# ultravideo/kvazzup

Measured on AMD Instinct MI355X. Metric: hevc_encode_decode_fps, higher is better.
Workload: dtype u8

## Files before the change

### kvazzup_amd/csrc/dec_parse.hip

```cpp
#include <chrono>
#include <cstdio>
#include <cstdlib>
#include <cstring>
#include "decoder.h"

namespace kvzx {

enum { PART_2Nx2N = 0, PART_2NxN, PART_Nx2N, PART_NxN, PART_2NxnU, PART_2NxnD, PART_nLx2N, PART_nRx2N };

namespace {

struct StateTabs { uint8_t next_mps[128], next_lps[128]; uint8_t next[128][2]; uint8_t lps[128][4]; uint32_t lpsn[128][4]; };
const StateTabs &state_tabs()
{
  static const StateTabs t = [] {
    StateTabs t;
    for (int s = 0; s < 128; s++) {
      int st = s >> 1, mps = s & 1;
      t.next_mps[s] = (uint8_t)(((st < 62 ? st + 1 : st) << 1) | mps);
      t.next_lps[s] = (uint8_t)((kNextLps[st] << 1) | (st == 0 ? mps ^ 1 : mps));
      t.next[s][0] = t.next_mps[s]; t.next[s][1] = t.next_lps[s];
      for (int q = 0; q < 4; q++) { t.lps[s][q] = kRangeLps[st][q]; const int n = __builtin_clz((uint32_t)kRangeLps[st][q]) - 23; t.lpsn[s][q] = ((uint32_t)kRangeLps[st][q] << n) | ((uint32_t)n << 16) | ((uint32_t)kRangeLps[st][q] << 24); }
    }
    return t;
  }();
  return t;
}
struct CabacRegs {
  const uint8_t *p = nullptr, *end = nullptr;
  uint64_t value = 0; int bits = 0;
  uint32_t range = 510; uint32_t past = 0;
  const StateTabs *st = nullptr;
  uint16_t *ctx = nullptr;
  static __attribute__((noinline)) uint32_t word_tail(const uint8_t *p, const uint8_t *end) { uint32_t w = 0; for (int i = 0; i < 4; i++) w = (w << 8) | (p + i < end ? p[i] : 0u); return w; }
  __attribute__((always_inline)) inline uint32_t word()
  {
    uint32_t w;
    if (__builtin_expect(p + 4 <= end, 1)) { memcpy(&w, p, 4); w = __builtin_bswap32(w); }
    else { w = word_tail(p, end); past++; }
    p += 4;
    return w;
  }
  __attribute__((always_inline)) inline void refill() { if (__builtin_expect(bits < 16, 0)) { value = (value << 32) | word(); bits += 32; } }
  bool overrun() const { return past > 3; }
  __attribute__((always_inline)) inline int bin(int ci)
  {
    const uint32_t s = ctx[ci];
    const uint32_t e = st->lpsn[s][(range >> 6) & 3];
    const uint32_t rmps = range - (e >> 24);
    const uint64_t scaled = (uint64_t)rmps << bits;
    const bool isl = value >= scaled;
    value -= isl ? scaled : 0;
    const uint32_t nm = (rmps >> 8) ^ 1u;
    range = isl ? (e & 0x1ffu) : (rmps << nm);
    bits -= (int)(isl ? ((e >> 16) & 15u) : nm);
    ctx[ci] = st->next[s][isl];
    refill();
    return (int)((s & 1u) ^ (uint32_t)isl);
  }
  __attribute__((always_inline)) inline int bypass()
  {
    bits--;
    const uint64_t scaled = (uint64_t)range << bits;
    int b = 0;
    if (value >= scaled) { value -= scaled; b = 1; }
    refill();
    return b;
  }
  __attribute__((always_inline)) inline uint32_t bypass_bits(int n)
  {
    uint32_t v = 0;
    while (n > 0) {
      const int m = n > 16 ? 16 : n;
      if (m <= 2) { for (int i = 0; i < m; i++) v = (v << 1) | (uint32_t)bypass(); }
      else {
        bits -= m;
        const uint64_t scaled = (uint64_t)range << bits;
        const uint64_t q = value / scaled;
        value -= q * scaled;
        v = (v << m) | (uint32_t)(q & 0xffffu);
        refill();
      }
      n -= m;
    }
    return v;
  }
  __attribute__((always_inline)) inline int terminate()
  {
    range -= 2;
    if (value >= ((uint64_t)range << bits)) return 1;
    if (range < 256) { range <<= 1; bits--; }
    refill();
    return 0;
  }
};
struct CabacDec : CabacRegs {
  const uint8_t *buf = nullptr;
  uint16_t ctx_store[CTX_COUNT];
  CabacDec() { ctx = ctx_store; }
  CabacDec(const CabacDec &) = delete;
  void load_ctx(const uint8_t *src) { for (int i = 0; i < CTX_COUNT; i++) ctx_store[i] = src[i]; }
  void save_ctx(uint8_t *dst) const { for (int i = 0; i < CTX_COUNT; i++) dst[i] = (uint8_t)ctx_store[i]; }
  void start(const uint8_t *b, size_t l)
  {
    buf = b; p = b; end = b + l; past = 0; st = &state_tabs(); range = 510; ctx = ctx_store;
    value = word(); bits = 32 - 9;
    refill();
  }
  size_t bytes_consumed() const { const size_t consumed_bits = (size_t)(p - buf) * 8 - (size_t)bits; return (consumed_bits + 7) >> 3; }
};

std::atomic<long> g_yields{0};

void parse_sao(CabacDec &c, SaoParams &p, const SaoParams *left, const SaoParams *up, bool luma, bool chroma)
{
  memset(&p, 0, sizeof(p));
  if (left && c.bin(CTX_SAO_MERGE)) { p = *left; return; }
  if (up && c.bin(CTX_SAO_MERGE)) { p = *up; return; }
  for (int ci = 0; ci < 3; ci++) {
    if (!(ci ? chroma : luma)) continue;
    if (ci < 2) p.type[ci] = (uint8_t)(c.bin(CTX_SAO_TYPE) ? (c.bypass() ? 2 : 1) : 0);
    else { p.type[2] = p.type[1]; p.eo_class[2] = p.eo_class[1]; }
    if (!p.type[ci]) continue;
    int a[4];
    for (int i = 0; i < 4; i++) { a[i] = 0; while (a[i] < 7 && c.bypass()) a[i]++; }
    if (p.type[ci] == 1) {
      for (int i = 0; i < 4; i++) if (a[i] && c.bypass()) a[i] = -a[i];
      p.band_pos[ci] = (uint8_t)c.bypass_bits(5);
    } else {
      if (ci < 2) p.eo_class[ci] = (uint8_t)c.bypass_bits(2);
      a[2] = -a[2]; a[3] = -a[3];
    }
    for (int i = 0; i < 4; i++) p.offset[ci][i] = (int8_t)a[i];
  }
}

__attribute__((noinline)) uint32_t sig_flag_run(CabacRegs &cr, const uint8_t *pk, int base, int k0)
{
  CabacRegs c = cr;
  uint32_t sig = 0;
  for (int k = k0; k >= 1; k--) sig |= (uint32_t)c.bin(base + pk[k]) << k;
  cr.p = c.p; cr.value = c.value; cr.bits = c.bits; cr.range = c.range; cr.past = c.past;
  return sig;
}
__attribute__((noinline)) uint32_t greater1_run(CabacRegs &cr, int ctx_base, int n, int *c1_io)
{
  CabacRegs c = cr;
  uint32_t g = 0; int c1 = *c1_io;
  for (int j = 0; j < n; j++) {
    const int g1 = c.bin(ctx_base + c1);
    g |= (uint32_t)g1 << j;
    if (g1) c1 = 0; else if (c1 > 0 && c1 < 3) c1++;
  }
  *c1_io = c1;
  cr.p = c.p; cr.value = c.value; cr.bits = c.bits; cr.range = c.range; cr.past = c.past;
  return g;
}

__attribute__((always_inline)) inline bool parse_residual_regs(CabacRegs &c, int log2, int cidx, int scan_idx, bool sign_hiding, bool ts_enabled, int *tskip, std::vector<uint32_t> &out)
{
  const ScanTabs &S = scan_tabs();
  const int n = 1 << log2, sbl = log2 - 2, nsb = 1 << sbl;
  const uint8_t *SX = S.x[scan_idx][sbl], *SY = S.y[scan_idx][sbl], *PX = S.x[scan_idx][2], *PY = S.y[scan_idx][2];
  uint8_t csbf[8][8]; memset(csbf, 0, sizeof(csbf));
  *tskip = (ts_enabled && log2 == 2) ? c.bin(CTX_TS_FLAG + (cidx ? 1 : 0)) : 0;
  int pre[2];
  for (int d = 0; d < 2; d++) {
    int off, sh, mx = (log2 << 1) - 1, v = 0;
    if (cidx == 0) { off = 3 * (log2 - 2) + ((log2 - 1) >> 2); sh = (log2 + 1) >> 2; } else { off = 15; sh = log2 - 2; }
    while (v < mx && c.bin((d ? CTX_LAST_Y : CTX_LAST_X) + off + (v >> sh))) v++;
    pre[d] = v;
  }
  int lx = pre[0], ly = pre[1];
  if (lx > 3) { int nb = (lx >> 1) - 1; lx = (1 << nb) * (2 + (lx & 1)) + (int)c.bypass_bits(nb); }
  if (ly > 3) { int nb = (ly >> 1) - 1; ly = (1 << nb) * (2 + (ly & 1)) + (int)c.bypass_bits(nb); }
  if (scan_idx == 2) { int tt = lx; lx = ly; ly = tt; }
  if (lx >= n || ly >= n) return false;
  const int last_sb = S.inv[scan_idx][sbl][((ly >> 2) << sbl) | (lx >> 2)], last_pos = S.inv[scan_idx][2][((ly & 3) << 2) | (lx & 3)];
  int c1 = 1;
  for (int i = last_sb; i >= 0; i--) {
    const int xs = SX[i], ys = SY[i];
    int right = (xs < nsb - 1) ? csbf[ys][xs + 1] : 0, below = (ys < nsb - 1) ? csbf[ys + 1][xs] : 0, infer_dc = 0;
    if (i < last_sb && i > 0) { csbf[ys][xs] = (uint8_t)c.bin(CTX_CSBF + ((right | below) ? 1 : 0) + (cidx ? 2 : 0)); infer_dc = 1; }
    else csbf[ys][xs] = 1;
    if (!csbf[ys][xs]) continue;
    uint32_t sig = 0;
    if (i == last_sb) sig |= 1u << last_pos;
    const int prev_csbf = right | (below << 1);
    const uint8_t *pk = S.sigk[scan_idx][log2 == 2 ? 4 : prev_csbf];
    const int sig_base = CTX_SIG + (cidx ? 27 : 0);
    const int sig_off = log2 == 2 ? 0 : (cidx == 0 ? ((i > 0 ? 3 : 0) + ((log2 == 3) ? ((scan_idx == 0) ? 9 : 15) : 21)) : ((log2 == 3) ? 9 : 12));
    {
      const int k0 = (i == last_sb) ? last_pos - 1 : 15;
      const int base = sig_base + sig_off;
      if (k0 >= 1) sig |= sig_flag_run(c, pk, base, k0);
      if (k0 >= 0) {
        if (infer_dc && !(sig >> 1)) sig |= 1u;
        else sig |= (uint32_t)c.bin((i == 0 && log2 != 2) ? sig_base : base + pk[0]);
      }
    }
    if (!sig) continue;
    int ctx_set = (i > 0 && cidx == 0) ? 2 : 0;
    if (c1 == 0) ctx_set++;
    c1 = 1;
    int pos[16], lev[16], nsig = 0, g1idx = -1;
    for (uint32_t m = sig; m;) { const int k = 31 - __builtin_clz(m); pos[nsig++] = k; m &= ~(1u << k); }
    for (int j = 0; j < nsig; j++) lev[j] = 1;
    {
      const uint32_t g = greater1_run(c, CTX_GT1 + (cidx ? 16 : 0) + ctx_set * 4, nsig < 8 ? nsig : 8, &c1);
      if (g) { g1idx = __builtin_ctz(g); for (uint32_t m = g; m; m &= m - 1) lev[__builtin_ctz(m)] = 2; }
    }
    if (g1idx >= 0 && c.bin(CTX_GT2 + (cidx ? 4 : 0) + ctx_set)) lev[g1idx] = 3;
    const bool hidden = sign_hiding && (pos[0] - pos[nsig - 1] > 3);
    const int nsigns = hidden ? nsig - 1 : nsig;
    uint32_t signs = c.bypass_bits(nsigns) << (nsig - nsigns);
    int rice = 0, sum = 0;
    for (int j = 0; j < nsig; j++) {
      int base = (j < 8) ? ((j == g1idx) ? 3 : 2) : 1;
      if (lev[j] == base) {
        int prefix = 0;
        while (prefix < 32 && c.bypass()) prefix++;
        if (prefix - 3 + rice > 16) return false;
        int rem = prefix <= 3 ? (prefix << rice) + (int)c.bypass_bits(rice)
                              : (((1 << (prefix - 3)) + 3 - 1) << rice) + (int)c.bypass_bits(prefix - 3 + rice);
        lev[j] = base + rem;
        if (lev[j] > 3 * (1 << rice)) rice = imin(rice + 1, 4);
      }
      sum += lev[j];
    }
    if (hidden && (sum & 1)) signs |= 1u;
    const size_t o0 = out.size();
    out.resize(o0 + (size_t)nsig);
    uint32_t *dst = out.data() + o0;
    for (int j = 0; j < nsig; j++) {
      const int v = ((signs >> (nsig - 1 - j)) & 1) ? -lev[j] : lev[j];
      const int xp = PX[pos[j]], yp = PY[pos[j]];
      dst[j] = (uint32_t)((((ys << 2) + yp) * n + (xs << 2) + xp) << 16) | ((uint32_t)clip3(-32768, 32767, v) & 0xffffu);
    }
    if (c.overrun()) return false;
  }
  return !c.overrun();
}

bool parse_residual(CabacDec &cd, int log2, int cidx, int scan_idx, bool sign_hiding, bool ts_enabled, int *tskip, std::vector<uint32_t> &out)
{
  CabacRegs c = cd;
  const bool ok = parse_residual_regs(c, log2, cidx, scan_idx, sign_hiding, ts_enabled, tskip, out);
  static_cast<CabacRegs &>(cd) = c;
  return ok;
}

struct MvCand { int mvx, mvy, ref_idx; };

struct SliceParser {
  Decoder::PicJob &job; Decoder::SubOut &out;
  const DecSps &sps; const DecPps &pps; const SliceHdr &sh;
  CabacDec c;
  const int w, h, b4w, b8w, ctbl, mincb, wc, hc;
  B4Rec *b4; uint8_t *pm, *ctd, *im;
  int ref_y0 = -(1 << 30), ref_y1 = 1 << 30;
  int tile_y0 = 0, tile_y1 = 1 << 30, tile_x0 = 0, tile_x1 = 1 << 30;
  const uint8_t *slice_of = nullptr; int cur_slice = 0;
  int slice_qp = 26;
  int err = 0;
  int qp_y = 0, qp_y_pred = 0, last_qp_y = 0, cu_qp_delta_val = 0, log2_qg = 6; bool qp_delta_coded = false;
  int cu_pred_mode = 0, part_mode = 0, max_trafo_depth = 0, intra_modes[4] = {0, 0, 0, 0}, chroma_mode = 0; bool intra_split = false;
  uint32_t ctu_intra_mask = 0;

  SliceParser(Decoder::PicJob &j, Decoder::SubOut &o, int pw)
      : job(j), out(o), sps(*j.sps), pps(j.pps), sh(j.sh), w(j.sps->width), h(j.sps->height), b4w(pw / 4), b8w(pw / 8), ctbl(j.sps->ctb_log2), mincb(j.sps->min_cb_log2), wc(j.sps->wc()),
        hc(j.sps->hc()), b4(j.b4), pm(j.pred_mode.data()), ctd(j.ct_depth.data()), im(j.intra_mode.data())
  { log2_qg = ctbl - pps.qp_delta_depth; }

  inline int bi(int x, int y) const { return (y >> 2) * b4w + (x >> 2); }
  inline int b8(int x, int y) const { return (y >> 3) * b8w + (x >> 3); }
  inline bool avail(int, int, int xn, int yn) const
  {
    return xn >= tile_x0 && yn >= tile_y0 && xn < w && yn < h && yn < tile_y1 && xn < tile_x1 && pm[b8(xn, yn)] != PM_NONE && (!slice_of || slice_of[(yn >> ctbl) * wc + (xn >> ctbl)] == cur_slice);
  }
  void fill_cu8(uint8_t *arr, int x0, int y0, int n, int v)
  {
    const int cols = imin(n, w - x0) >> 3;
    for (int y = y0; y < y0 + n && y < h; y += 8) memset(arr + b8(x0, y), v, (size_t)cols);
  }
  void fill_u8(uint8_t *arr, int x0, int y0, int bw, int bh, int v)
  {
    const int cols = imin(bw, w - x0) >> 2;
    for (int y = y0; y < y0 + bh && y < h; y += 4) memset(arr + bi(x0, y), v, (size_t)cols);
  }
  bool cu_edges_done = false;
  int cu_bypass = 0;
  void fill_recs(int x0, int y0, int bw, int bh, const B4Rec &r, bool cu_edges = false)
  {
    uint64_t v; memcpy(&v, &r, 8);
    const int cols = imin(bw, w - x0) >> 2;
    if (!cu_edges) { for (int y = y0; y < y0 + bh && y < h; y += 4) { uint64_t *p = (uint64_t *)&b4[bi(x0, y)]; for (int i = 0; i < cols; i++) p[i] = v; } return; }
    B4Rec e = r;
    e.flags |= B4_EDGE_V | B4_TU_V; uint64_t vl; memcpy(&vl, &e, 8);
    e.flags = r.flags | B4_EDGE_H | B4_TU_H; uint64_t vt; memcpy(&vt, &e, 8);
    e.flags |= B4_EDGE_V | B4_TU_V; uint64_t vc; memcpy(&vc, &e, 8);
    for (int y = y0; y < y0 + bh && y < h; y += 4) {
      uint64_t *p = (uint64_t *)&b4[bi(x0, y)];
      const bool top = y == y0;
      if (cols > 0) p[0] = top ? vc : vl;
      for (int i = 1; i < cols; i++) p[i] = top ? vt : v;
    }
    cu_edges_done = true;
  }
  void emit_tu(const DecTu &td)
  {
    const int X = td.plane ? td.x * 2 : td.x, Y = td.plane ? td.y * 2 : td.y;
    if (ctbl == 6) {
      TuRange &r = job.region[(Y >> 5) * (b4w >> 3) + (X >> 5)];
      if (!r.count) r.first = (uint32_t)out.tus.size();
      r.count++;
    }
    out.tus.push_back(td);
  }

  bool pb_avail(int xcb, int ycb, int ncbs, int xpb, int ypb, int npbw, int npbh, int part_idx, int xn, int yn) const
  {
    const bool same_cb = xcb <= xn && ycb <= yn && xcb + ncbs > xn && ycb + ncbs > yn;
    bool a;
    if (!same_cb) a = avail(xpb, ypb, xn, yn);
    else a = !((npbw << 1) == ncbs && (npbh << 1) == ncbs && part_idx == 1 && (ycb + npbh <= yn) && (xcb + npbw > xn));
    if (a && pm[b8(xn, yn)] == PM_INTRA) a = false;
    return a;
  }
  static bool same_motion(const B4Rec &a, const B4Rec &b) { return a.ref_idx == b.ref_idx && a.mvx == b.mvx && a.mvy == b.mvy; }

  inline int list_poc(int L, int idx) const { return L ? job.ref_poc1[idx & 15] : job.ref_poc[idx & 15]; }
  inline bool list_lt(int L, int idx) const { return (L ? job.ref_lt1[idx & 15] : job.ref_lt[idx & 15]) != 0; }
  static void scale_by(int &mvx, int &mvy, int td_, int tb_)
  {
    const int td = clip3(-128, 127, td_), tb = clip3(-128, 127, tb_);
    if (td == 0) return;
    const int tx = (16384 + (iabs(td) >> 1)) / td, dsf = clip3(-4096, 4095, (tb * tx + 32) >> 6);
    const int px = dsf * mvx, py = dsf * mvy;
    mvx = clip3(-32768, 32767, (px < 0 ? -1 : 1) * ((iabs(px) + 127) >> 8));
    mvy = clip3(-32768, 32767, (py < 0 ? -1 : 1) * ((iabs(py) + 127) >> 8));
  }
  bool temporal_mv(int xpb, int ypb, int npbw, int npbh, int X, int ref_idx, int &mvx, int &mvy)
  {
    ColMotion *col = job.col.get();
    if (!col) return false;
    const int cy = ypb >> ctbl;
    if (cy < col->hc) {
      std::atomic<uint8_t> &d = col->row_done[(size_t)cy];
      int spins = 0;
      while (!d.load(std::memory_order_acquire)) { if (++spins < 2000) __builtin_ia32_pause(); else std::this_thread::yield(); }
    }
    const int cand[2][2] = {{xpb + npbw, ypb + npbh}, {xpb + (npbw >> 1), ypb + (npbh >> 1)}};
    for (int k = 0; k < 2; k++) {
      int x = cand[k][0], y = cand[k][1];
      if (k == 0 && !((ypb >> ctbl) == (y >> ctbl) && y < h && x < w)) continue;
      x >>= 4; y >>= 4;
      if (x >= col->w16 || y >= col->h16) continue;
      const ColMotion::Mv &m = col->mv[(size_t)y * col->w16 + x];
      if (!m.used) continue;
      const int L = m.used == 2 ? 1 : (m.used == 1 ? 0 : (job.no_backward ? X : sh.collocated_from_l0));
      const bool cur_lt = list_lt(X, ref_idx);
      if ((((m.lt >> L) & 1) != 0) != cur_lt) continue;
      const int col_diff = col->poc - m.ref_poc[L], cur_diff = sh.poc - list_poc(X, ref_idx);
      mvx = m.mv[L][0]; mvy = m.mv[L][1];
      if (!cur_lt && col_diff != cur_diff && col_diff != 0) scale_by(mvx, mvy, col_diff, cur_diff);
      return true;
    }
    return false;
  }

  void merge_candidates(int xcb, int ycb, int ncbs, int xpb, int ypb, int npbw, int npbh, int part_idx, int pmode, MvCand *cand, int want)
  {
    const int lvl = pps.par_mrg_level;
    int n = 0;
    if (lvl > 2 && ncbs == 8) { xpb = xcb; ypb = ycb; npbw = npbh = ncbs; part_idx = 0; pmode = PART_2Nx2N; }
    auto par = [&](int xn, int yn) { return ((xpb >> lvl) == (xn >> lvl)) && ((ypb >> lvl) == (yn >> lvl)); };
    const int xa1 = xpb - 1, ya1 = ypb + npbh - 1, xb1 = xpb + npbw - 1, yb1 = ypb - 1, xb0 = xpb + npbw, yb0 = ypb - 1;
    const int xa0 = xpb - 1, ya0 = ypb + npbh, xb2 = xpb - 1, yb2 = ypb - 1;
    const bool part1 = part_idx == 1;
    const bool nbA1 = pb_avail(xcb, ycb, ncbs, xpb, ypb, npbw, npbh, part_idx, xa1, ya1) && !par(xa1, ya1) &&
                      !(part1 && (pmode == PART_Nx2N || pmode == PART_nLx2N || pmode == PART_nRx2N));
    if (want == 0 && nbA1) { const B4Rec &m = b4[bi(xa1, ya1)]; cand[0].mvx = m.mvx; cand[0].mvy = m.mvy; cand[0].ref_idx = m.ref_idx; return; }
    const bool nbB1 = pb_avail(xcb, ycb, ncbs, xpb, ypb, npbw, npbh, part_idx, xb1, yb1) && !par(xb1, yb1) &&
                      !(part1 && (pmode == PART_2NxN || pmode == PART_2NxnU || pmode == PART_2NxnD));
    const bool nbB0 = pb_avail(xcb, ycb, ncbs, xpb, ypb, npbw, npbh, part_idx, xb0, yb0) && !par(xb0, yb0);
    const bool nbA0 = pb_avail(xcb, ycb, ncbs, xpb, ypb, npbw, npbh, part_idx, xa0, ya0) && !par(xa0, ya0);
    const bool nbB2 = pb_avail(xcb, ycb, ncbs, xpb, ypb, npbw, npbh, part_idx, xb2, yb2) && !par(xb2, yb2);
    const B4Rec zero = B4Rec();
    const B4Rec &A1 = nbA1 ? b4[bi(xa1, ya1)] : zero, &B1 = nbB1 ? b4[bi(xb1, yb1)] : zero, &B0 = nbB0 ? b4[bi(xb0, yb0)] : zero;
    const B4Rec &A0 = nbA0 ? b4[bi(xa0, ya0)] : zero, &B2 = nbB2 ? b4[bi(xb2, yb2)] : zero;
    const bool avA1 = nbA1, avB1 = nbB1 && !(nbA1 && same_motion(A1, B1)), avB0 = nbB0 && !(nbB1 && same_motion(B1, B0));
    const bool avA0 = nbA0 && !(nbA1 && same_motion(A1, A0));
    const bool avB2 = nbB2 && !(nbA1 && same_motion(A1, B2)) && !(nbB1 && same_motion(B1, B2)) && ((int)avA0 + avA1 + avB0 + avB1 != 4);
    const int maxc = sh.max_merge;
    auto add = [&](const B4Rec &m) { if (n < maxc) { cand[n].mvx = m.mvx; cand[n].mvy = m.mvy; cand[n].ref_idx = m.ref_idx; n++; } };
    if (avA1) add(A1);
    if (avB1) add(B1);
    if (avB0) add(B0);
    if (avA0) add(A0);
    if (avB2) add(B2);
    if (n < maxc) { int tx, ty; if (temporal_mv(xpb, ypb, npbw, npbh, 0, 0, tx, ty)) { cand[n].mvx = tx; cand[n].mvy = ty; cand[n].ref_idx = 0; n++; } }
    for (int zi = 0; n < maxc; n++, zi++) { cand[n].mvx = cand[n].mvy = 0; cand[n].ref_idx = zi < sh.num_ref_idx ? zi : 0; }
  }

  void scale_mv(int &mvx, int &mvy, int ref_a, int ref_target) const
  {
    const int td = clip3(-128, 127, sh.poc - job.ref_poc[ref_a]), tb = clip3(-128, 127, sh.poc - job.ref_poc[ref_target]);
    if (td == 0) return;
    const int tx = (16384 + (iabs(td) >> 1)) / td, dsf = clip3(-4096, 4095, (tb * tx + 32) >> 6);
    const int px = dsf * mvx, py = dsf * mvy;
    mvx = clip3(-32768, 32767, (px < 0 ? -1 : 1) * ((iabs(px) + 127) >> 8));
    mvy = clip3(-32768, 32767, (py < 0 ? -1 : 1) * ((iabs(py) + 127) >> 8));
  }

  void amvp_candidates(int xcb, int ycb, int ncbs, int xpb, int ypb, int npbw, int npbh, int part_idx, int ref_idx, int cand[2][2])
  {
    const int xa[2] = {xpb - 1, xpb - 1}, ya[2] = {ypb + npbh, ypb + npbh - 1};
    const int xb[3] = {xpb + npbw, xpb + npbw - 1, xpb - 1}, yb[3] = {ypb - 1, ypb - 1, ypb - 1};
    bool avA[2], avB[3];
    for (int k = 0; k < 2; k++) avA[k] = pb_avail(xcb, ycb, ncbs, xpb, ypb, npbw, npbh, part_idx, xa[k], ya[k]);
    for (int k = 0; k < 3; k++) avB[k] = pb_avail(xcb, ycb, ncbs, xpb, ypb, npbw, npbh, part_idx, xb[k], yb[k]);
    const bool is_scaled = avA[0] || avA[1];
    bool flagA = false, flagB = false; int ax = 0, ay = 0, bx = 0, by = 0;
    const int target = job.ref_poc[ref_idx];
    const bool tlt = job.ref_lt[ref_idx & 15] != 0;
    for (int k = 0; k < 2 && !flagA; k++) if (avA[k]) { const B4Rec &m = b4[bi(xa[k], ya[k])]; if (job.ref_poc[m.ref_idx & 15] == target) { flagA = true; ax = m.mvx; ay = m.mvy; } }
    for (int k = 0; k < 2 && !flagA; k++) if (avA[k]) { const B4Rec &m = b4[bi(xa[k], ya[k])]; if ((job.ref_lt[m.ref_idx & 15] != 0) != tlt) continue; flagA = true; ax = m.mvx; ay = m.mvy; if (!tlt) scale_mv(ax, ay, m.ref_idx & 15, ref_idx); }
    for (int k = 0; k < 3 && !flagB; k++) if (avB[k]) { const B4Rec &m = b4[bi(xb[k], yb[k])]; if (job.ref_poc[m.ref_idx & 15] == target) { flagB = true; bx = m.mvx; by = m.mvy; } }
    if (!is_scaled && flagB) { flagA = true; ax = bx; ay = by; }
    if (!is_scaled) {
      flagB = false;
      for (int k = 0; k < 3 && !flagB; k++) if (avB[k]) {
        const B4Rec &m = b4[bi(xb[k], yb[k])];
        if ((job.ref_lt[m.ref_idx & 15] != 0) != tlt) continue;
        flagB = true; bx = m.mvx; by = m.mvy;
        if (!tlt && job.ref_poc[m.ref_idx & 15] != target) scale_mv(bx, by, m.ref_idx & 15, ref_idx);
      }
    }
    int n = 0;
    if (flagA) { cand[n][0] = ax; cand[n][1] = ay; n++; }
    if (flagB && !(flagA && ax == bx && ay == by)) { cand[n][0] = bx; cand[n][1] = by; n++; }
    if (n < 2) { int tx, ty; if (temporal_mv(xpb, ypb, npbw, npbh, 0, ref_idx, tx, ty)) { cand[n][0] = tx; cand[n][1] = ty; n++; } }
    for (; n < 2; n++) cand[n][0] = cand[n][1] = 0;
  }

  typedef Decoder::PicJob::MvF MvF;
  MvF *mvf = nullptr;
  static bool same_motion_b(const MvF &a, const MvF &b)
  {
    if (a.ref[0] != b.ref[0] || a.ref[1] != b.ref[1]) return false;
    if (a.ref[0] >= 0 && (a.mv[0][0] != b.mv[0][0] || a.mv[0][1] != b.mv[0][1])) return false;
    if (a.ref[1] >= 0 && (a.mv[1][0] != b.mv[1][0] || a.mv[1][1] != b.mv[1][1])) return false;
    return true;
  }
  void merge_candidates_b(int xcb, int ycb, int ncbs, int xpb, int ypb, int npbw, int npbh, int part_idx, int pmode, MvF *cand)
  {
    const int lvl = pps.par_mrg_level;
    int n = 0;
    if (lvl > 2 && ncbs == 8) { xpb = xcb; ypb = ycb; npbw = npbh = ncbs; part_idx = 0; pmode = PART_2Nx2N; }
    auto par = [&](int xn, int yn) { return ((xpb >> lvl) == (xn >> lvl)) && ((ypb >> lvl) == (yn >> lvl)); };
    const int xa1 = xpb - 1, ya1 = ypb + npbh - 1, xb1 = xpb + npbw - 1, yb1 = ypb - 1, xb0 = xpb + npbw, yb0 = ypb - 1;
    const int xa0 = xpb - 1, ya0 = ypb + npbh, xb2 = xpb - 1, yb2 = ypb - 1;
    const bool part1 = part_idx == 1;
    const bool nbA1 = pb_avail(xcb, ycb, ncbs, xpb, ypb, npbw, npbh, part_idx, xa1, ya1) && !par(xa1, ya1) &&
                      !(part1 && (pmode == PART_Nx2N || pmode == PART_nLx2N || pmode == PART_nRx2N));
    const bool nbB1 = pb_avail(xcb, ycb, ncbs, xpb, ypb, npbw, npbh, part_idx, xb1, yb1) && !par(xb1, yb1) &&
                      !(part1 && (pmode == PART_2NxN || pmode == PART_2NxnU || pmode == PART_2NxnD));
    const bool nbB0 = pb_avail(xcb, ycb, ncbs, xpb, ypb, npbw, npbh, part_idx, xb0, yb0) && !par(xb0, yb0);
    const bool nbA0 = pb_avail(xcb, ycb, ncbs, xpb, ypb, npbw, npbh, part_idx, xa0, ya0) && !par(xa0, ya0);
    const bool nbB2 = pb_avail(xcb, ycb, ncbs, xpb, ypb, npbw, npbh, part_idx, xb2, yb2) && !par(xb2, yb2);
    MvF zero; memset(&zero, 0, sizeof(zero)); zero.ref[0] = zero.ref[1] = -1;
    const MvF &A1 = nbA1 ? mvf[bi(xa1, ya1)] : zero, &B1 = nbB1 ? mvf[bi(xb1, yb1)] : zero, &B0 = nbB0 ? mvf[bi(xb0, yb0)] : zero;
    const MvF &A0 = nbA0 ? mvf[bi(xa0, ya0)] : zero, &B2 = nbB2 ? mvf[bi(xb2, yb2)] : zero;
    const bool avA1 = nbA1, avB1 = nbB1 && !(nbA1 && same_motion_b(A1, B1)), avB0 = nbB0 && !(nbB1 && same_motion_b(B1, B0));
    const bool avA0 = nbA0 && !(nbA1 && same_motion_b(A1, A0));
    const bool avB2 = nbB2 && !(nbA1 && same_motion_b(A1, B2)) && !(nbB1 && same_motion_b(B1, B2)) && ((int)avA0 + avA1 + avB0 + avB1 != 4);
    const int maxc = sh.max_merge;
    auto add = [&](const MvF &m) { if (n < maxc) cand[n++] = m; };
    if (avA1) add(A1);
    if (avB1) add(B1);
    if (avB0) add(B0);
    if (avA0) add(A0);
    if (avB2) add(B2);
    if (n < maxc) {
      int x0 = 0, y0 = 0, x1 = 0, y1 = 0;
      const bool f0 = temporal_mv(xpb, ypb, npbw, npbh, 0, 0, x0, y0), f1 = temporal_mv(xpb, ypb, npbw, npbh, 1, 0, x1, y1);
      if (f0 || f1) {
        MvF &t = cand[n++];
        t.mv[0][0] = (int16_t)x0; t.mv[0][1] = (int16_t)y0; t.ref[0] = f0 ? 0 : -1;
        t.mv[1][0] = (int16_t)x1; t.mv[1][1] = (int16_t)y1; t.ref[1] = f1 ? 0 : -1;
      }
    }
    if (n > 1 && n < maxc) {
      static const uint8_t l0c[12] = {0, 1, 0, 2, 1, 2, 0, 3, 1, 3, 2, 3}, l1c[12] = {1, 0, 2, 0, 2, 1, 3, 0, 3, 1, 3, 2};
      const int norig = n;
      for (int comb = 0; comb < norig * (norig - 1) && n < maxc; comb++) {
        const MvF &p0 = cand[l0c[comb]], &p1 = cand[l1c[comb]];
        if (p0.ref[0] < 0 || p1.ref[1] < 0) continue;
        if (list_poc(0, p0.ref[0]) == list_poc(1, p1.ref[1]) && p0.mv[0][0] == p1.mv[1][0] && p0.mv[0][1] == p1.mv[1][1]) continue;
        MvF &t = cand[n++];
        t.mv[0][0] = p0.mv[0][0]; t.mv[0][1] = p0.mv[0][1]; t.ref[0] = p0.ref[0];
        t.mv[1][0] = p1.mv[1][0]; t.mv[1][1] = p1.mv[1][1]; t.ref[1] = p1.ref[1];
      }
    }
    const int nrefs = imin(sh.num_ref_idx, sh.num_ref_idx1);
    for (int zi = 0; n < maxc; n++, zi++) { MvF &t = cand[n]; memset(&t, 0, sizeof(t)); t.ref[0] = t.ref[1] = (int8_t)(zi < nrefs ? zi : 0); }
  }
  void amvp_candidates_b(int xcb, int ycb, int ncbs, int xpb, int ypb, int npbw, int npbh, int part_idx, int X, int ref_idx, int cand[2][2])
  {
    const int xa[2] = {xpb - 1, xpb - 1}, ya[2] = {ypb + npbh, ypb + npbh - 1};
    const int xb[3] = {xpb + npbw, xpb + npbw - 1, xpb - 1}, yb[3] = {ypb - 1, ypb - 1, ypb - 1};
    bool avA[2], avB[3];
    for (int k = 0; k < 2; k++) avA[k] = pb_avail(xcb, ycb, ncbs, xpb, ypb, npbw, npbh, part_idx, xa[k], ya[k]);
    for (int k = 0; k < 3; k++) avB[k] = pb_avail(xcb, ycb, ncbs, xpb, ypb, npbw, npbh, part_idx, xb[k], yb[k]);
    const bool is_scaled = avA[0] || avA[1];
    bool flagA = false, flagB = false; int ax = 0, ay = 0, bx = 0, by = 0;
    const int target = list_poc(X, ref_idx), Y = X ^ 1;
    auto same_pic = [&](const MvF &m, int &vx, int &vy) {
      for (int L : {X, Y}) if (m.ref[L] >= 0 && list_poc(L, m.ref[L]) == target) { vx = m.mv[L][0]; vy = m.mv[L][1]; return true; }
      return false;
    };
    const bool tlt = list_lt(X, ref_idx);
    auto any_pic = [&](const MvF &m, int &vx, int &vy) {
      for (int L : {X, Y}) if (m.ref[L] >= 0 && list_lt(L, m.ref[L]) == tlt) {
        vx = m.mv[L][0]; vy = m.mv[L][1];
        const int poc = list_poc(L, m.ref[L]);
        if (!tlt && poc != target) scale_by(vx, vy, sh.poc - poc, sh.poc - target);
        return true;
      }
      return false;
    };
    for (int k = 0; k < 2 && !flagA; k++) if (avA[k]) flagA = same_pic(mvf[bi(xa[k], ya[k])], ax, ay);
    for (int k = 0; k < 2 && !flagA; k++) if (avA[k]) flagA = any_pic(mvf[bi(xa[k], ya[k])], ax, ay);
    for (int k = 0; k < 3 && !flagB; k++) if (avB[k]) flagB = same_pic(mvf[bi(xb[k], yb[k])], bx, by);
    if (!is_scaled && flagB) { flagA = true; ax = bx; ay = by; }
    if (!is_scaled) {
      flagB = false;
      for (int k = 0; k < 3 && !flagB; k++) if (avB[k]) flagB = any_pic(mvf[bi(xb[k], yb[k])], bx, by);
    }
    int n = 0;
    if (flagA) { cand[n][0] = ax; cand[n][1] = ay; n++; }
    if (flagB && !(flagA && ax == bx && ay == by)) { cand[n][0] = bx; cand[n][1] = by; n++; }
    if (n < 2) { int tx, ty; if (temporal_mv(xpb, ypb, npbw, npbh, X, ref_idx, tx, ty)) { cand[n][0] = tx; cand[n][1] = ty; n++; } }
    for (; n < 2; n++) cand[n][0] = cand[n][1] = 0;
  }
  int parse_ref_idx(int num_active)
  {
    int ref_idx = 0;
    const int mx = num_active - 1;
    while (ref_idx < mx && ref_idx < 2 && c.bin(CTX_REF_IDX + ref_idx)) ref_idx++;
    if (ref_idx == 2) while (ref_idx < mx && c.bypass()) ref_idx++;
    return ref_idx;
  }
  void parse_mvd(int &dx, int &dy)
  {
    const int g0x = c.bin(CTX_MVD_GT0), g0y = c.bin(CTX_MVD_GT0);
    const int g1x = g0x ? c.bin(CTX_MVD_GT1) : 0, g1y = g0y ? c.bin(CTX_MVD_GT1) : 0;
    dx = mvd_abs(g0x, g1x); if (g0x && c.bypass()) dx = -dx;
    dy = mvd_abs(g0y, g1y); if (g0y && c.bypass()) dy = -dy;
  }
  void prediction_unit_b(int xcb, int ycb, int ncbs, int xp, int yp, int bw, int bh, int part_idx, bool skip, int *merge_out)
  {
    const int merge = skip ? 1 : c.bin(CTX_MERGE_FLAG);
    if (merge_out) *merge_out = merge;
    MvF m; memset(&m, 0, sizeof(m)); m.ref[0] = m.ref[1] = -1;
    if (merge) {
      int idx = 0;
      if (sh.max_merge > 1 && c.bin(CTX_MERGE_IDX)) { idx = 1; while (idx < sh.max_merge - 1 && c.bypass()) idx++; }
      MvF cand[5];
      merge_candidates_b(xcb, ycb, ncbs, xp, yp, bw, bh, part_idx, part_mode, cand);
      m = cand[idx];
      if (m.ref[0] >= 0 && m.ref[1] >= 0 && bw + bh == 12) { m.ref[1] = -1; m.mv[1][0] = m.mv[1][1] = 0; }
    } else {
      int idc;
      if (bw + bh != 12 && c.bin(CTX_INTER_PRED_IDC + ctd[b8(xcb, ycb)])) idc = 2;
      else idc = c.bin(CTX_INTER_PRED_IDC + 4);
      for (int X = 0; X < 2; X++) {
        if (idc == 1 - X) continue;
        const int na = X ? sh.num_ref_idx1 : sh.num_ref_idx;
        const int ref_idx = na > 1 ? parse_ref_idx(na) : 0;
        int dx = 0, dy = 0;
        if (!(X == 1 && sh.mvd_l1_zero && idc == 2)) parse_mvd(dx, dy);
        const int mvp = c.bin(CTX_MVP_FLAG);
        if (ref_idx >= (X ? job.nref1 : job.nref)) { err = DEC_ERR_INVALID; return; }
        int cand[2][2];
        amvp_candidates_b(xcb, ycb, ncbs, xp, yp, bw, bh, part_idx, X, ref_idx, cand);
        m.mv[X][0] = (int16_t)(uint16_t)(cand[mvp][0] + dx); m.mv[X][1] = (int16_t)(uint16_t)(cand[mvp][1] + dy);
        m.ref[X] = (int8_t)ref_idx;
      }
    }
    if ((m.ref[0] < 0 && m.ref[1] < 0) || m.ref[0] >= job.nref || m.ref[1] >= job.nref1) { err = DEC_ERR_INVALID; return; }
    if (ref_y1 != (1 << 30) || ref_y0 != -(1 << 30)) { err = DEC_ERR_UNSUPPORTED; return; }
    const int P = m.ref[0] >= 0 ? 0 : 1;
    const bool bi = m.ref[0] >= 0 && m.ref[1] >= 0;
    const bool wtd = sh.weighted && (((m.ref[0] >= 0) && ((sh.wt_explicit >> m.ref[0]) & 1)) || ((m.ref[1] >= 0) && ((sh.wt_explicit >> (16 + m.ref[1])) & 1)));
    B4Rec r; r.mvx = m.mv[P][0]; r.mvy = m.mv[P][1]; r.ref_idx = m.ref[P]; r.flags = (uint8_t)((cu_bypass ? B4_BYPASS : 0) | (bi ? B4_BI : 0) | (wtd ? B4_WT : 0)); r.qp_y = (int8_t)qp_y;
    r.slot = P ? job.ref_slot1[m.ref[1]] : job.ref_slot[m.ref[0]];
    fill_recs(xp, yp, bw, bh, r, bw == ncbs && bh == ncbs);
    B4L1 x; x.mvx = m.mv[1][0]; x.mvy = m.mv[1][1]; x.slot = bi ? job.ref_slot1[m.ref[1]] : 0; x.pad[0] = (uint8_t)(P * 16 + m.ref[P]); x.pad[1] = (uint8_t)(bi ? 16 + m.ref[1] : 0); x.pad[2] = 0;
    const int cols = imin(bw, w - xp) >> 2;
    const bool ext = bi || wtd;
    for (int y = yp; y < yp + bh && y < h; y += 4) { const int i0 = bi_(xp, y); for (int i = 0; i < cols; i++) { mvf[i0 + i] = m; if (ext) job.b4x[(size_t)(i0 + i)] = x; } }
    if (ext) if (!job.any_bi.load(std::memory_order_relaxed)) job.any_bi.store(1, std::memory_order_relaxed);
    if (bw != ncbs || bh != ncbs) {
      for (int i = 0; i < bh && yp + i < h; i += 4) b4[bi_(xp, yp + i)].flags |= B4_EDGE_V;
      for (int i = 0; i < bw && xp + i < w; i += 4) b4[bi_(xp + i, yp)].flags |= B4_EDGE_H;
    }
  }
  inline int bi_(int x, int y) const { return (y >> 2) * b4w + (x >> 2); }

  int mvd_abs(int gt0, int gt1)
  {
    if (!gt0) return 0;
    if (!gt1) return 1;
    int k = 1, v = 0;
    while (k < 17 && c.bypass()) { v += 1 << k; k++; }
    if (k >= 17) { err = DEC_ERR_INVALID; return 0; }
    return v + (int)c.bypass_bits(k) + 2;
  }

  void prediction_unit(int xcb, int ycb, int ncbs, int xp, int yp, int bw, int bh, int part_idx, bool skip, int *merge_out)
  {
    if (sh.is_b) { prediction_unit_b(xcb, ycb, ncbs, xp, yp, bw, bh, part_idx, skip, merge_out); return; }
    const int merge = skip ? 1 : c.bin(CTX_MERGE_FLAG);
    if (merge_out) *merge_out = merge;
    int mvx, mvy, ref_idx = 0;
    if (merge) {
      int idx = 0;
      if (sh.max_merge > 1 && c.bin(CTX_MERGE_IDX)) { idx = 1; while (idx < sh.max_merge - 1 && c.bypass()) idx++; }
      MvCand cand[5];
      merge_candidates(xcb, ycb, ncbs, xp, yp, bw, bh, part_idx, part_mode, cand, idx);
      mvx = cand[idx].mvx; mvy = cand[idx].mvy; ref_idx = cand[idx].ref_idx;
    } else {
      if (sh.num_ref_idx > 1) {
        const int mx = sh.num_ref_idx - 1;
        while (ref_idx < mx && ref_idx < 2 && c.bin(CTX_REF_IDX + ref_idx)) ref_idx++;
        if (ref_idx == 2) while (ref_idx < mx && c.bypass()) ref_idx++;
      }
      const int g0x = c.bin(CTX_MVD_GT0), g0y = c.bin(CTX_MVD_GT0);
      const int g1x = g0x ? c.bin(CTX_MVD_GT1) : 0, g1y = g0y ? c.bin(CTX_MVD_GT1) : 0;
      int dx = mvd_abs(g0x, g1x); if (g0x && c.bypass()) dx = -dx;
      int dy = mvd_abs(g0y, g1y); if (g0y && c.bypass()) dy = -dy;
      const int mvp = c.bin(CTX_MVP_FLAG);
      int cand[2][2];
      amvp_candidates(xcb, ycb, ncbs, xp, yp, bw, bh, part_idx, ref_idx, cand);
      mvx = (int16_t)(uint16_t)(cand[mvp][0] + dx); mvy = (int16_t)(uint16_t)(cand[mvp][1] + dy);
    }
    if (ref_idx < 0 || ref_idx >= job.nref) { err = DEC_ERR_INVALID; ref_idx = 0; }
    if (ref_y1 != (1 << 30) || ref_y0 != -(1 << 30)) {
      const int fy = mvy & 3, fc = mvy & 7;
      const int top = imin(yp + (mvy >> 2) - (fy ? 3 : 0), 2 * ((yp >> 1) + (mvy >> 3) - (fc ? 1 : 0)));
      const int bot = imax(yp + bh + (mvy >> 2) + (fy ? 4 : 0), 2 * ((yp >> 1) + (bh >> 1) + (mvy >> 3) + (fc ? 2 : 0)));
      if (top < ref_y0 || bot > ref_y1) err = DEC_ERR_UNSUPPORTED;
    }
    B4Rec r; r.mvx = (int16_t)mvx; r.mvy = (int16_t)mvy; r.ref_idx = (int8_t)ref_idx; r.flags = (uint8_t)((cu_bypass ? B4_BYPASS : 0) | ((sh.weighted && ((sh.wt_explicit >> ref_idx) & 1)) ? B4_WT : 0)); r.qp_y = (int8_t)qp_y; r.slot = job.ref_slot[ref_idx];
    fill_recs(xp, yp, bw, bh, r, bw == ncbs && bh == ncbs);
    if (r.flags & B4_WT) {
      B4L1 x; x.mvx = 0; x.mvy = 0; x.slot = 0; x.pad[0] = (uint8_t)ref_idx; x.pad[1] = x.pad[2] = 0;
      const int cols = imin(bw, w - xp) >> 2;
      for (int y = yp; y < yp + bh && y < h; y += 4) { const int i0 = bi(xp, y); for (int i = 0; i < cols; i++) job.b4x[(size_t)(i0 + i)] = x; }
      if (!job.any_bi.load(std::memory_order_relaxed)) job.any_bi.store(1, std::memory_order_relaxed);
    }
    if (bw != ncbs || bh != ncbs) {
      for (int i = 0; i < bh && yp + i < h; i += 4) b4[bi(xp, yp + i)].flags |= B4_EDGE_V;
      for (int i = 0; i < bw && xp + i < w; i += 4) b4[bi(xp + i, yp)].flags |= B4_EDGE_H;
    }
  }

  void transform_unit(int x0, int y0, int xbase, int ybase, int log2, int blk, int cbf_luma, int cbf_cb, int cbf_cr, int cbf_cb_parent, int cbf_cr_parent)
  {
    const bool intra = cu_pred_mode == PM_INTRA;
    const bool chroma_here = log2 > 2, chroma_parent = log2 == 2 && blk == 3;
    const int ccb = chroma_here ? cbf_cb : (chroma_parent ? cbf_cb_parent : 0), ccr = chroma_here ? cbf_cr : (chroma_parent ? cbf_cr_parent : 0);
    const bool cbf_chroma_any = log2 > 2 ? (cbf_cb || cbf_cr) : (cbf_cb_parent || cbf_cr_parent);
    if ((cbf_luma || cbf_chroma_any) && pps.cu_qp_delta && !qp_delta_coded) {
      int v = 0;
      while (v < 5 && c.bin(CTX_CU_QP_DELTA + (v ? 1 : 0))) v++;
      if (v == 5) { int k = 0; while (k < 16 && c.bypass()) { v += 1 << k; k++; } if (k >= 16) { err = DEC_ERR_INVALID; return; } v += (int)c.bypass_bits(k); }
      if (v && c.bypass()) v = -v;
      if (v < -26 || v > 25) { err = DEC_ERR_INVALID; return; }
      qp_delta_coded = true; cu_qp_delta_val = v;
      qp_y = (qp_y_pred + v + 52) % 52;
    }
    const int n = 1 << log2;
    DecTu td; td.pad = 0;
    const int lmode = intra ? im[bi(x0, y0)] : 0;
    if (intra || cbf_luma) {
      td.x = (uint16_t)x0; td.y = (uint16_t)y0; td.plane = 0; td.log2 = (uint8_t)log2; td.mode = (uint8_t)lmode; td.qp = (int8_t)qp_y;
      td.flags = (uint8_t)((intra ? TU_INTRA : 0) | ((intra && log2 == 2) ? TU_DST : 0) | (cu_bypass ? TU_BYPASS : 0));
      td.offset = (uint32_t)out.levels.size(); td.count = 0;
      if (cbf_luma) {
        int ts;
        if (!parse_residual(c, log2, 0, intra_scan_idx(intra, log2, 0, lmode), pps.sign_hiding != 0 && !cu_bypass, pps.tskip != 0 && !cu_bypass, &ts, out.levels)) { err = DEC_ERR_INVALID; return; }
        td.count = (uint16_t)(out.levels.size() - td.offset);
        if (ts) td.flags |= TU_TSKIP;
        for (int y = y0; y < y0 + n && y < h; y += 4) for (int x = x0; x < x0 + n && x < w; x += 4) b4[bi(x, y)].flags |= B4_NZ;
      }
      emit_tu(td);
      if (intra) ctu_intra_mask |= 1u;
    }
    if (chroma_here || chroma_parent) {
      const int cx = (chroma_here ? x0 : xbase) >> 1, cy = (chroma_here ? y0 : ybase) >> 1, clog2 = chroma_here ? log2 - 1 : 2;
      for (int ci = 1; ci <= 2; ci++) {
        const int cbf = ci == 1 ? ccb : ccr;
        if (!intra && !cbf) continue;
        td.x = (uint16_t)cx; td.y = (uint16_t)cy; td.plane = (uint8_t)ci; td.log2 = (uint8_t)clog2; td.mode = (uint8_t)chroma_mode;
        td.qp = (int8_t)kChromaQp[clip3(0, 57, qp_y + (ci == 1 ? sh.cb_qp_offset : sh.cr_qp_offset))];
        td.flags = (uint8_t)((intra ? TU_INTRA : 0) | (cu_bypass ? TU_BYPASS : 0));
        td.offset = (uint32_t)out.levels.size(); td.count = 0;
        if (cbf) {
          int ts;
          if (!parse_residual(c, clog2, ci, intra_scan_idx(intra, clog2, ci, chroma_mode), pps.sign_hiding != 0 && !cu_bypass, pps.tskip != 0 && !cu_bypass, &ts, out.levels)) { err = DEC_ERR_INVALID; return; }
          td.count = (uint16_t)(out.levels.size() - td.offset);
          if (ts) td.flags |= TU_TSKIP;
        }
        emit_tu(td);
        if (intra) ctu_intra_mask |= 1u << ci;
      }
    }
  }

  void transform_tree(int x0, int y0, int xbase, int ybase, int log2, int depth, int blk, int cbf_cb_parent, int cbf_cr_parent)
  {
    if (err) return;
    int split;
    if (log2 <= 5 && log2 > 2 && depth < max_trafo_depth && !(intra_split && depth == 0)) split = c.bin(CTX_SPLIT_TRANSFORM + 5 - log2);
    else {
      const bool inter_split = sps.th_depth_inter == 0 && cu_pred_mode == PM_INTER && part_mode != PART_2Nx2N && depth == 0;
      split = (log2 > imin(5, ctbl) || (intra_split && depth == 0) || inter_split) ? 1 : 0;
    }
    int cbf_cb = 0, cbf_cr = 0;
    if (log2 > 2) {
      if (depth == 0 || cbf_cb_parent) cbf_cb = c.bin(CTX_CBF_CHROMA + depth);
      if (depth == 0 || cbf_cr_parent) cbf_cr = c.bin(CTX_CBF_CHROMA + depth);
    } else { cbf_cb = cbf_cb_parent; cbf_cr = cbf_cr_parent; }
    if (split) {
      if (log2 <= 2) { err = DEC_ERR_INVALID; return; }
      const int hh = 1 << (log2 - 1);
      transform_tree(x0, y0, x0, y0, log2 - 1, depth + 1, 0, cbf_cb, cbf_cr);
      transform_tree(x0 + hh, y0, x0, y0, log2 - 1, depth + 1, 1, cbf_cb, cbf_cr);
      transform_tree(x0, y0 + hh, x0, y0, log2 - 1, depth + 1, 2, cbf_cb, cbf_cr);
      transform_tree(x0 + hh, y0 + hh, x0, y0, log2 - 1, depth + 1, 3, cbf_cb, cbf_cr);
    } else {
      int cbf_luma = 1;
      if (cu_pred_mode == PM_INTRA || depth != 0 || cbf_cb || cbf_cr) cbf_luma = c.bin(CTX_CBF_LUMA + (depth == 0 ? 1 : 0));
      if (depth > 0) {
        const int n = 1 << log2;
        for (int i = 0; i < n; i += 4) {
          if (y0 + i < h) b4[bi(x0, y0 + i)].flags |= B4_EDGE_V | B4_TU_V;
          if (x0 + i < w) b4[bi(x0 + i, y0)].flags |= B4_EDGE_H | B4_TU_H;
        }
      }
      transform_unit(x0, y0, xbase, ybase, log2, blk, cbf_luma, log2 > 2 ? cbf_cb : 0, log2 > 2 ? cbf_cr : 0, cbf_cb_parent, cbf_cr_parent);
    }
  }

  void coding_unit(int x0, int y0, int log2cb, int depth)
  {
    const int n = 1 << log2cb;
    int skip = 0;
    cu_bypass = pps.tq_bypass ? c.bin(CTX_TQ_BYPASS) : 0;
    if (!sh.is_intra) {
      const int l = avail(x0, y0, x0 - 1, y0) && pm[b8(x0 - 1, y0)] == PM_SKIP, a = avail(x0, y0, x0, y0 - 1) && pm[b8(x0, y0 - 1)] == PM_SKIP;
      skip = c.bin(CTX_SKIP + l + a);
    }
    part_mode = PART_2Nx2N; intra_split = false; cu_edges_done = false;
    int rqt_root_cbf = 1, merge_2nx2n = 0;
    fill_cu8(ctd, x0, y0, n, depth);
    qp_y = (qp_y_pred + cu_qp_delta_val + 52) % 52;
    if (skip) {
      cu_pred_mode = PM_INTER;
      fill_cu8(pm, x0, y0, n, PM_SKIP);
      prediction_unit(x0, y0, n, x0, y0, n, n, 0, true, nullptr);
      rqt_root_cbf = 0;
      if (!job.any_inter) job.any_inter = true;
    } else {
      cu_pred_mode = PM_INTRA;
      if (!sh.is_intra) cu_pred_mode = c.bin(CTX_PRED_MODE) ? PM_INTRA : PM_INTER;
      if (cu_pred_mode != PM_INTRA || log2cb == mincb) {
        if (cu_pred_mode == PM_INTRA) part_mode = c.bin(CTX_PART_MODE) ? PART_2Nx2N : PART_NxN;
        else if (c.bin(CTX_PART_MODE)) part_mode = PART_2Nx2N;
        else if (log2cb == mincb) {
          if (c.bin(CTX_PART_MODE + 1)) part_mode = PART_2NxN;
          else if (log2cb == 3) part_mode = PART_Nx2N;
          else part_mode = c.bin(CTX_PART_MODE + 2) ? PART_Nx2N : PART_NxN;
        }
        else if (!sps.amp) part_mode = c.bin(CTX_PART_MODE + 1) ? PART_2NxN : PART_Nx2N;
        else {
          const int horiz = c.bin(CTX_PART_MODE + 1);
          if (c.bin(CTX_PART_MODE + 3)) part_mode = horiz ? PART_2NxN : PART_Nx2N;
          else { const int b = c.bypass(); part_mode = horiz ? (b ? PART_2NxnD : PART_2NxnU) : (b ? PART_nRx2N : PART_nLx2N); }
        }
      }
      fill_cu8(pm, x0, y0, n, cu_pred_mode);
      if (cu_pred_mode == PM_INTRA && part_mode == PART_2Nx2N && sps.pcm_depth[0] && log2cb >= sps.pcm_min_log2 && log2cb <= sps.pcm_max_log2 && c.terminate()) {
        const uint8_t *q = c.buf + c.bytes_consumed();
        const size_t need = ((size_t)n * n * sps.pcm_depth[0] + (size_t)n * n / 2 * sps.pcm_depth[1]) / 8;
        if (q > c.end || need > (size_t)(c.end - q)) { err = DEC_ERR_INVALID; return; }
        BitReader pr(q, need);
        for (int ci = 0; ci < 3; ci++) {
          const int shp = ci ? 1 : 0, m = n >> shp, depth = sps.pcm_depth[ci ? 1 : 0];
          DecTu td; td.pad = 0; td.x = (uint16_t)(x0 >> shp); td.y = (uint16_t)(y0 >> shp); td.plane = (uint8_t)ci; td.log2 = (uint8_t)(log2cb - shp); td.mode = 35; td.qp = 0;
          td.flags = (uint8_t)(TU_INTRA | TU_BYPASS); td.offset = (uint32_t)out.levels.size();
          for (int y = 0; y < m; y++)
            for (int x = 0; x < m; x++) { const uint32_t v = pr.get(depth) << (8 - depth); if (v) out.levels.push_back((uint32_t)((y * m + x) << 16) | v); }
          td.count = (uint16_t)(out.levels.size() - td.offset);
          emit_tu(td);
          ctu_intra_mask |= 1u << ci;
        }
        c.start(q + need, (size_t)(c.end - (q + need)));
        fill_u8(im, x0, y0, n, n, 1);
        B4Rec r; r.mvx = 0; r.mvy = 0; r.ref_idx = -1; r.flags = (uint8_t)((cu_bypass || sps.pcm_no_filter) ? B4_BYPASS : 0); r.qp_y = (int8_t)qp_y; r.slot = 0;
        fill_recs(x0, y0, n, n, r, true);
        if (!job.any_intra) job.any_intra = true;
        rqt_root_cbf = 0;
      } else
      if (cu_pred_mode == PM_INTRA) {
        intra_split = part_mode == PART_NxN;
        const int parts = intra_split ? 2 : 1, pb = n / parts;
        int prev[4], k = 0;
        for (int j = 0; j < parts * parts; j++) prev[j] = c.bin(CTX_PREV_INTRA);
        for (int j = 0; j < parts; j++)
          for (int i = 0; i < parts; i++, k++) {
            const int xp = x0 + i * pb, yp = y0 + j * pb;
            int ca = 1, cb = 1;
            if (avail(xp, yp, xp - 1, yp) && pm[b8(xp - 1, yp)] == PM_INTRA) ca = im[bi(xp - 1, yp)];
            if (avail(xp, yp, xp, yp - 1) && pm[b8(xp, yp - 1)] == PM_INTRA && (yp - 1) >= ((yp >> ctbl) << ctbl)) cb = im[bi(xp, yp - 1)];
            int cand[3];
            if (ca == cb) {
              if (ca < 2) { cand[0] = 0; cand[1] = 1; cand[2] = 26; }
              else { cand[0] = ca; cand[1] = 2 + ((ca + 29) % 32); cand[2] = 2 + ((ca - 2 + 1) % 32); }
            } else {
              cand[0] = ca; cand[1] = cb;
              cand[2] = (ca != 0 && cb != 0) ? 0 : ((ca != 1 && cb != 1) ? 1 : 26);
            }
            int mode;
            if (prev[k]) { int idx = 0; if (c.bypass()) { idx = 1; if (c.bypass()) idx = 2; } mode = cand[idx]; }
            else {
              mode = (int)c.bypass_bits(5);
              int t;
              if (cand[0] > cand[1]) { t = cand[0]; cand[0] = cand[1]; cand[1] = t; }
              if (cand[0] > cand[2]) { t = cand[0]; cand[0] = cand[2]; cand[2] = t; }
              if (cand[1] > cand[2]) { t = cand[1]; cand[1] = cand[2]; cand[2] = t; }
              for (int q = 0; q < 3; q++) if (mode >= cand[q]) mode++;
            }
            intra_modes[k] = mode;
            fill_u8(im, xp, yp, pb, pb, mode);
          }
        int icpm = 4;
        if (c.bin(CTX_CHROMA_MODE)) icpm = (int)c.bypass_bits(2);
        static const int cm[4] = {0, 26, 10, 1};
        if (icpm == 4) chroma_mode = intra_modes[0];
        else { chroma_mode = cm[icpm]; if (chroma_mode == intra_modes[0]) chroma_mode = 34; }
        B4Rec r; r.mvx = 0; r.mvy = 0; r.ref_idx = -1; r.flags = (uint8_t)(cu_bypass ? B4_BYPASS : 0); r.qp_y = (int8_t)qp_y; r.slot = 0;
        fill_recs(x0, y0, n, n, r, true);
        if (!job.any_intra) job.any_intra = true;
      } else {
        const int hh = n / 2, q = n / 4; int mf = 0;
        switch (part_mode) {
          case PART_2Nx2N: prediction_unit(x0, y0, n, x0, y0, n, n, 0, false, &merge_2nx2n); break;
          case PART_2NxN: prediction_unit(x0, y0, n, x0, y0, n, hh, 0, false, &mf); prediction_unit(x0, y0, n, x0, y0 + hh, n, hh, 1, false, &mf); break;
          case PART_Nx2N: prediction_unit(x0, y0, n, x0, y0, hh, n, 0, false, &mf); prediction_unit(x0, y0, n, x0 + hh, y0, hh, n, 1, false, &mf); break;
          case PART_2NxnU: prediction_unit(x0, y0, n, x0, y0, n, q, 0, false, &mf); prediction_unit(x0, y0, n, x0, y0 + q, n, n - q, 1, false, &mf); break;
          case PART_2NxnD: prediction_unit(x0, y0, n, x0, y0, n, n - q, 0, false, &mf); prediction_unit(x0, y0, n, x0, y0 + n - q, n, q, 1, false, &mf); break;
          case PART_nLx2N: prediction_unit(x0, y0, n, x0, y0, q, n, 0, false, &mf); prediction_unit(x0, y0, n, x0 + q, y0, n - q, n, 1, false, &mf); break;
          case PART_NxN:
            for (int k = 0; k < 4; k++) prediction_unit(x0, y0, n, x0 + (k & 1) * hh, y0 + (k >> 1) * hh, hh, hh, k, false, &mf);
            break;
          default: prediction_unit(x0, y0, n, x0, y0, n - q, n, 0, false, &mf); prediction_unit(x0, y0, n, x0 + n - q, y0, q, n, 1, false, &mf); break;
        }
        if (!(part_mode == PART_2Nx2N && merge_2nx2n)) rqt_root_cbf = c.bin(CTX_RQT_ROOT_CBF);
        if (!job.any_inter) job.any_inter = true;
      }
    }
    if (err) return;
    if (!cu_edges_done) {
      B4Rec *const r0 = &b4[bi(x0, y0)];
      const int rows = (imin(n, h - y0) + 3) >> 2, cols = (imin(n, w - x0) + 3) >> 2;
      for (int i = 0; i < rows; i++) r0[(size_t)i * b4w].flags |= B4_EDGE_V | B4_TU_V;
      for (int i = 0; i < cols; i++) r0[i].flags |= B4_EDGE_H | B4_TU_H;
    }
    const int qp_before = qp_y;
    if (rqt_root_cbf) {
      max_trafo_depth = cu_pred_mode == PM_INTRA ? sps.th_depth_intra + (intra_split ? 1 : 0) : sps.th_depth_inter;
      transform_tree(x0, y0, x0, y0, log2cb, 0, 0, 0, 0);
    }
    if (qp_y != qp_before)
      for (int y = y0; y < y0 + n && y < h; y += 4) for (int x = x0; x < x0 + n && x < w; x += 4) b4[bi(x, y)].qp_y = (int8_t)qp_y;
    last_qp_y = qp_y;
  }

  void coding_quadtree(int x0, int y0, int log2cb, int depth)
  {
    if (err) return;
    const int n = 1 << log2cb;
    int split;
    if (x0 + n <= w && y0 + n <= h && log2cb > mincb) {
      const int l = avail(x0, y0, x0 - 1, y0) && ctd[b8(x0 - 1, y0)] > depth, a = avail(x0, y0, x0, y0 - 1) && ctd[b8(x0, y0 - 1)] > depth;
      split = c.bin(CTX_SPLIT_CU + l + a);
    } else split = log2cb > mincb;
    if (pps.cu_qp_delta && log2cb >= log2_qg) {
      qp_delta_coded = false; cu_qp_delta_val = 0;
      int qa = last_qp_y, qb = last_qp_y;
      if (avail(x0, y0, x0 - 1, y0) && ((x0 - 1) >> ctbl) == (x0 >> ctbl)) qa = b4[bi(x0 - 1, y0)].qp_y;
      if (avail(x0, y0, x0, y0 - 1) && ((y0 - 1) >> ctbl) == (y0 >> ctbl)) qb = b4[bi(x0, y0 - 1)].qp_y;
      qp_y_pred = (qa + qb + 1) >> 1;
    }
    if (split) {
      const int hh = n >> 1;
      coding_quadtree(x0, y0, log2cb - 1, depth + 1);
      if (x0 + hh < w) coding_quadtree(x0 + hh, y0, log2cb - 1, depth + 1);
      if (y0 + hh < h) coding_quadtree(x0, y0 + hh, log2cb - 1, depth + 1);
      if (x0 + hh < w && y0 + hh < h) coding_quadtree(x0 + hh, y0 + hh, log2cb - 1, depth + 1);
    } else coding_unit(x0, y0, log2cb, depth);
  }
};

}

int Decoder::parse_substream(PicJob &job, int sub, const uint8_t *data, size_t len, SubOut &out)
{
  SliceParser sp(job, out, pw_);
  tl("row0", sub);
  struct RowEnd { int s; ~RowEnd() { tl("row1", s); } } row_end_{sub};
  if (job.sh.is_b) sp.mvf = job.mvf.data();
  const int wc = sp.wc;
  const DecPps &pps = job.pps; const SliceHdr &sh = job.sh;
  const bool wpp = pps.wpp != 0;
  const PicJob::SubGeom g = job.geom[(size_t)sub];
  const int first_cy = g.cy0, ncy = g.cy1 - g.cy0, cx0 = g.cx0, cx1 = g.cx1, tw = cx1 - cx0, cols = pps.tile_cols;
  auto tile_starts_at = [&](int cy) { return cy == g.tile_cy0; };
  auto tile_ends_at = [&](int cy) { return cy + 1 == g.tile_cy1; };
  int seen_above = 0;
  auto wait_above = [&](int cy, int need) {
    if (!wpp || tile_starts_at(cy)) return true;
    if (need > tw) need = tw;
    if (seen_above < need) {
      std::atomic<int> &p = job.row_progress[(size_t)(cy - 1) * cols + g.tc].v;
      int spins = 0;
      while ((seen_above = p.load(std::memory_order_acquire)) < need) {
        if (++spins < 2000) __builtin_ia32_pause(); else { g_yields.fetch_add(1, std::memory_order_relaxed); std::this_thread::yield(); }
      }
    }
    return seen_above < (1 << 29);
  };
  const int init_type = sh.is_intra ? 0 : (sh.is_b ? (sh.cabac_init_flag ? 1 : 2) : (sh.cabac_init_flag ? 2 : 1));
  CabacDec &c = sp.c;
  const bool free_slices = !job.ctb_cut.empty();
  const bool scan = job.scan_gaps && cols == 1 && (!wpp || free_slices);
  bool skipping = false;
  size_t first_off = 0;
  if (scan && free_slices) {
    const int a0 = first_cy * wc + cx0;
    const uint8_t cut0 = job.ctb_cut[(size_t)a0];
    if (cut0 & 1) skipping = false;
    else if (a0 == 0) skipping = true;
    else if (cut0 & 2) { if (!wait_above(first_cy, tw)) return DEC_ERR_INVALID; skipping = job.miss_map[(size_t)a0 - 1] != 0; }
    else if (job.sub_start[(size_t)first_cy] == SIZE_MAX || job.row_seg_start[(size_t)first_cy] < 0) skipping = true;
    else {
      const int s0 = job.row_seg_start[(size_t)first_cy];
      if (!wait_above(first_cy, s0 / wc == first_cy - 1 ? imax(2, s0 % wc + 1) : 2)) return DEC_ERR_INVALID;
      skipping = job.miss_map[(size_t)s0] != 0;
    }
    if (wpp && !skipping) { first_off = job.sub_start[(size_t)first_cy]; if (first_off == SIZE_MAX || first_off >= len) return DEC_ERR_INVALID; }
  }
  c.start(data + first_off, len - first_off);
  sp.slice_qp = sh.slice_qp;
  if (free_slices) { sp.slice_of = job.ctb_slice.data(); sp.cur_slice = job.ctb_slice[(size_t)first_cy * wc + cx0]; sp.slice_qp = job.slice_qps[(size_t)sp.cur_slice]; }
  auto init_contexts = [&] { uint8_t init[CTX_COUNT]; cabac_init_contexts(init, init_type, sp.slice_qp); c.load_ctx(init); };
  if (skipping) init_contexts();
  else if (!wpp || tile_starts_at(first_cy) || tw < 2) init_contexts();
  else if (scan && !wait_above(first_cy, 2)) return DEC_ERR_INVALID;
  else if (free_slices && job.ctb_slice[(size_t)(first_cy - 1) * wc + cx0 + 1] != sp.cur_slice) {
    if (job.ctb_cut[(size_t)first_cy * wc + cx0] & 2) {
      if (!wait_above(first_cy, tw)) return DEC_ERR_INVALID;
      c.load_ctx(&job.ds_saved[(size_t)(first_cy - 1) * CTX_COUNT]);
    } else init_contexts();
  } else {
    if (!wait_above(first_cy, 2)) return DEC_ERR_INVALID;
    c.load_ctx(&job.wpp_saved[((size_t)(first_cy - 1) * cols + g.tc) * CTX_COUNT]);
  }
  sp.last_qp_y = sp.slice_qp;
  sp.tile_y0 = g.tile_cy0 << ctbl_; sp.tile_y1 = g.tile_cy1 << ctbl_; sp.tile_x0 = cx0 << ctbl_; sp.tile_x1 = cx1 << ctbl_;
  if (band_nrows_ > 0) {
    if (band_row0_ > 0) sp.ref_y0 = band_row0_ * 64 - 4;
    if (band_row0_ + band_nrows_ < (h_ + 63) / 64) sp.ref_y1 = (band_row0_ + band_nrows_) * 64;
  }
  ColMotion *own = job.own.get();
  auto mark_missing = [&](int ctu) {
    const int per = 1 << (ctbl_ - 2), b4w = pw_ / 4, mx = ctu % wc, my = ctu / wc;
    B4Rec none; memset(&none, 0, sizeof(none)); none.ref_idx = -1;
    for (int k = 0; k < per; k++) for (int x = 0; x < per; x++) job.b4[(size_t)(my * per + k) * b4w + mx * per + x] = none;
    job.ctu_tile[ctu] = 255; if (free_slices) job.ctb_slice[(size_t)ctu] = 255;
    memset(&job.sao[ctu], 0, sizeof(SaoParams));
    job.miss_map[(size_t)ctu] = 1;
    if (wpp) job.row_progress[(size_t)(ctu / wc) * cols + g.tc].v.store(ctu % wc - cx0 + 1, std::memory_order_release);
  };
  for (int cy = first_cy; cy < first_cy + ncy; cy++) {
    if (cy > first_cy && job.row_restart[(size_t)cy] != SIZE_MAX) {
      const uint8_t *q = job.rbsp.data() + job.data_off + job.row_restart[(size_t)cy];
      if (q < data || q >= data + len) return DEC_ERR_INVALID;
      c.start(q, (size_t)(data + len - q));
    }
    for (int cx = cx0; cx < cx1; cx++) {
      if (!wait_above(cy, cx - cx0 + 2)) return DEC_ERR_INVALID;
      const int ctu = cy * wc + cx;
      const uint8_t cut = free_slices ? job.ctb_cut[(size_t)ctu] : 0;
      if (skipping) {
        if (!(cut & 1)) { mark_missing(ctu); continue; }
        skipping = false;
      }
      if (cut & 3) {
        if (cx != cx0 || cy != first_cy) {
          const uint8_t *q = job.rbsp.data() + job.data_off + job.ctb_data[(size_t)ctu];
          if (q < data || q >= data + len) return DEC_ERR_INVALID;
          c.start(q, (size_t)(data + len - q));
        }
        if (cut & 1) {
          sp.cur_slice = job.ctb_slice[(size_t)ctu]; sp.slice_qp = job.slice_qps[(size_t)sp.cur_slice];
          init_contexts();
          sp.last_qp_y = sp.slice_qp;
        }
      }
      const uint32_t tu0 = (uint32_t)out.tus.size();
      sp.ctu_intra_mask = 0;
      if (!pps.cu_qp_delta) { sp.qp_y_pred = sp.slice_qp; sp.cu_qp_delta_val = 0; }
      if (sh.sao_luma || sh.sao_chroma) {
        SaoParams *s = &job.sao[ctu];
        const SaoParams *left = cx > cx0 ? s - 1 : nullptr, *up = (cy > 0 && !tile_starts_at(cy)) ? s - wc : nullptr;
        if (free_slices) { if (left && job.ctb_slice[(size_t)ctu - 1] != sp.cur_slice) left = nullptr; if (up && job.ctb_slice[(size_t)ctu - wc] != sp.cur_slice) up = nullptr; }
        parse_sao(c, *s, left, up, sh.sao_luma != 0, sh.sao_chroma != 0);
      }
      static const char *const ctu_dump = getenv("KVAZZUP_AMD_CTU_DUMP");
      std::chrono::steady_clock::time_point ctu_t0;
      if (__builtin_expect(ctu_dump != nullptr, 0)) ctu_t0 = std::chrono::steady_clock::now();
      sp.coding_quadtree(cx << ctbl_, cy << ctbl_, ctbl_, 0);
      if (__builtin_expect(ctu_dump != nullptr, 0)) {
        const long ns = (long)std::chrono::duration_cast<std::chrono::nanoseconds>(std::chrono::steady_clock::now() - ctu_t0).count();
        static FILE *const fp = fopen(ctu_dump, "w"); static std::mutex m;
        if (fp) { std::lock_guard<std::mutex> l(m); fprintf(fp, "%d %d %d %ld\n", job.sh.poc, cy, cx, ns); fflush(fp); }
      }
      if (sp.err) return sp.err;
      if (c.overrun()) return DEC_ERR_INVALID;
      job.ctu[ctu].first = tu0;
      job.ctu[ctu].count = ((uint32_t)out.tus.size() - tu0) | (sp.ctu_intra_mask << 24);
      if (out.tus.size() - tu0 >= (1u << 24)) return DEC_ERR_INVALID;
      if (wpp && cx == cx0 + 1) c.save_ctx(&job.wpp_saved[((size_t)cy * cols + g.tc) * CTX_COUNT]);
      if (((cut & 4) || scan) && wpp && free_slices && cx == cx1 - 1) c.save_ctx(&job.ds_saved[(size_t)cy * CTX_COUNT]);
      if (wpp) job.row_progress[(size_t)cy * cols + g.tc].v.store(cx - cx0 + 1, std::memory_order_release);
      const bool seg_last = free_slices ? (cut & 4) != 0 : cx == cx1 - 1 && (cols > 1 ? (cy == g.cy1 - 1 && job.seg_end_sub[(size_t)sub]) : job.seg_end_row[(size_t)cy] != 0);
      const int end = c.terminate();
      if (end != (seg_last ? 1 : 0)) {
        if (scan && end == 1 && !job.ambiguous_end) skipping = true;
        else return seg_last ? DEC_ERR_INVALID : (job.ambiguous_end ? DEC_SEG_ENDS_EARLY : DEC_ERR_UNSUPPORTED);
      }
      if (!skipping && !seg_last && cx == cx1 - 1 && (wpp || tile_ends_at(cy)) && !c.terminate()) return DEC_ERR_INVALID;
    }
    if (job.early_dst) {
      const size_t rowb = (size_t)(4 << (ctbl_ - 4)) * (pw_ / 4) * sizeof(B4Rec), off = (size_t)cy * rowb;
      if (hipSetDevice(device_) == hipSuccess && hipMemcpyAsync(job.early_dst + off, job.h_in + off, rowb, hipMemcpyHostToDevice, stream_up_) == hipSuccess)
        job.early_rows.fetch_add(1, std::memory_order_acq_rel);
    }
    const int per16 = 1 << (ctbl_ - 4);
    if (ConcealMotion *cm = job.cown.get()) {
      for (int y16 = cy * per16; y16 < (cy + 1) * per16 && y16 < cm->h16; y16++)
        for (int x16 = cx0 * per16; x16 < cx1 * per16 && x16 < cm->w16; x16++) {
          const size_t i4 = (size_t)(y16 * 4) * (pw_ / 4) + x16 * 4;
          const B4Rec &m = job.b4[i4];
          ConcealMotion::E &o = cm->e[(size_t)y16 * cm->w16 + x16];
          o.none = 1;
          if (m.ref_idx < 0) continue;
          if (sh.is_b) {
            const PicJob::MvF &f = job.mvf[i4];
            const int L = f.ref[0] >= 0 ? 0 : 1;
            if (f.ref[L] < 0) continue;
            o.mv[0] = f.mv[L][0]; o.mv[1] = f.mv[L][1]; o.ref_poc = L ? job.ref_poc1[f.ref[L] & 15] : job.ref_poc[f.ref[L] & 15]; o.lt = (L ? job.ref_lt1 : job.ref_lt)[f.ref[L] & 15] ? 1 : 0;
          } else { o.mv[0] = m.mvx; o.mv[1] = m.mvy; o.ref_poc = job.ref_poc[m.ref_idx & 15]; o.lt = job.ref_lt[m.ref_idx & 15] ? 1 : 0; }
          o.none = 0;
        }
    }
    if (!own) continue;
    for (int y16 = cy * per16; y16 < (cy + 1) * per16 && y16 < own->h16; y16++)
      for (int x16 = cx0 * per16; x16 < cx1 * per16 && x16 < own->w16; x16++) {
        const size_t i4 = (size_t)(y16 * 4) * (pw_ / 4) + x16 * 4;
        const B4Rec &m = job.b4[i4];
        ColMotion::Mv &o = own->mv[(size_t)y16 * own->w16 + x16];
        memset(&o, 0, sizeof(o));
        if (m.ref_idx < 0) continue;
        if (sh.is_b) {
          const PicJob::MvF &f = job.mvf[i4];
          for (int L = 0; L < 2; L++) if (f.ref[L] >= 0) { o.used |= (uint8_t)(1 << L); o.mv[L][0] = f.mv[L][0]; o.mv[L][1] = f.mv[L][1]; o.ref_poc[L] = L ? job.ref_poc1[f.ref[L] & 15] : job.ref_poc[f.ref[L] & 15]; if ((L ? job.ref_lt1 : job.ref_lt)[f.ref[L] & 15]) o.lt |= (uint8_t)(1 << L); }
        } else { o.used = 1; o.mv[0][0] = m.mvx; o.mv[0][1] = m.mvy; o.ref_poc[0] = job.ref_poc[m.ref_idx & 15]; o.lt = job.ref_lt[m.ref_idx & 15] ? 1 : 0; }
      }
    if (own->row_cols[(size_t)cy].fetch_add(1, std::memory_order_acq_rel) + 1 >= own->cols) own->row_done[(size_t)cy].store(1, std::memory_order_release);
  }
  return 0;
}

int Decoder::parse_job(PicJob &job, bool row_parallel)
{
  const uint8_t *data = job.rbsp.data() + job.data_off; const size_t len = job.data_len;
  const int wc = ctbs_in(w_, ctbl_), hc = ctbs_in(h_, ctbl_), nsub = (int)job.geom.size(), cols = job.pps.tile_cols;
  auto release_all = [&] { if (job.own) for (int r = 0; r < hc; r++) job.own->row_done[(size_t)r].store(1, std::memory_order_release); };
  std::vector<uint8_t> miss;
  int nrecv = nsub;
  const bool scan_rows = job.scan_gaps && job.pps.wpp != 0 && !job.ctb_cut.empty();
  if (job.scan_gaps) { job.missing.clear(); job.miss_map.assign((size_t)wc * hc, 0); }
  if (!job.missing.empty()) {
    miss.assign((size_t)wc * hc, 0);
    if (job.missing.size() != 1 || !job.pps.wpp || cols != 1 || nsub != hc || band_nrows_ > 0) { release_all(); return DEC_ERR_INVALID; }
    const int a = job.missing[0].first, n = job.missing[0].second;
    if (a <= 0 || a % wc != 0 || a + n != wc * hc) { release_all(); return DEC_ERR_INVALID; }
    memset(miss.data() + a, 1, (size_t)n);
    nrecv = a / wc;
  }
  if ((int)job.sub_start.size() != nrecv) { release_all(); return DEC_ERR_INVALID; }
  for (int r = 0; r < nrecv; r++) if (job.sub_start[(size_t)r] >= len && !(scan_rows && job.sub_start[(size_t)r] == SIZE_MAX)) { release_all(); return DEC_ERR_INVALID; }
  if (scan_rows && (int)job.row_seg_start.size() != hc) { release_all(); return DEC_ERR_INVALID; }
  job.subs.resize((size_t)nsub);
  for (auto &r : job.subs) { r.levels.clear(); r.tus.clear(); r.rc = 0; }
  job.wpp_saved.resize((size_t)hc * cols * CTX_COUNT);
  if (!job.row_progress || job.row_progress_n < hc * cols) { job.row_progress.reset(new Progress[(size_t)hc * cols]); job.row_progress_n = hc * cols; }
  for (int r = 0; r < hc * cols; r++) job.row_progress[(size_t)r].v.store(0, std::memory_order_relaxed);
  memset(job.region, 0, (size_t)(pw_ / 32) * (ph_ / 32) * sizeof(TuRange));
  memset(job.ctu, 0, nctb() * sizeof(TuRange));
  memset(job.pred_mode.data(), PM_NONE, job.pred_mode.size());
  auto skip_row = [&](int cy) {
    const int per = 1 << (ctbl_ - 2), b4w = pw_ / 4;
    B4Rec none; memset(&none, 0, sizeof(none)); none.ref_idx = -1;
    for (int k = 0; k < per; k++) for (int x = 0; x < b4w; x++) job.b4[(size_t)(cy * per + k) * b4w + x] = none;
    memset(job.ctu_tile + (size_t)cy * wc, 255, (size_t)wc);
    memset(&job.sao[(size_t)cy * wc], 0, (size_t)wc * sizeof(SaoParams));
    job.subs[(size_t)cy].rc = 0;
    job.row_progress[(size_t)cy].v.store(wc, std::memory_order_release);
    if (ColMotion *own = job.own.get()) {
      const int per16 = 1 << (ctbl_ - 4);
      for (int y16 = cy * per16; y16 < (cy + 1) * per16 && y16 < own->h16; y16++) memset(&own->mv[(size_t)y16 * own->w16], 0, (size_t)own->w16 * sizeof(ColMotion::Mv));
      own->row_cols[(size_t)cy].store((uint8_t)own->cols, std::memory_order_release); own->row_done[(size_t)cy].store(1, std::memory_order_release);
    }
  };
  auto one = [&](int r) {
    if (r >= nrecv) { skip_row(job.geom[(size_t)r].cy0); return; }
    if (band_nrows_ > 0 && (job.geom[(size_t)r].cy0 < band_row0_ || job.geom[(size_t)r].cy1 > band_row0_ + band_nrows_)) { job.subs[(size_t)r].rc = 0; return; }
    size_t start = job.sub_start[(size_t)r], end = (r + 1 < nrecv) ? job.sub_start[(size_t)r + 1] : len;
    if (scan_rows) { start = 0; end = len; }
    int rc = end > start ? parse_substream(job, r, data + start, end - start, job.subs[(size_t)r]) : DEC_ERR_INVALID;
    job.subs[(size_t)r].rc = rc;
    if (rc < 0 && job.pps.wpp) job.row_progress[(size_t)job.geom[(size_t)r].cy0 * cols + job.geom[(size_t)r].tc].v.store(1 << 30, std::memory_order_release);
    if (rc < 0) release_all();
  };
  if (row_parallel && nsub > 1) {
    if (!pool_) {
      const char *e = getenv("KVAZZUP_AMD_PARSE_THREADS");
      if (e) parse_threads_ = atoi(e) < 1 ? 1 : atoi(e);
      else if (frame_threads_ > 1 && parse_threads_ > 8) parse_threads_ = 8;
      pool_.reset(new OrderedPool(parse_threads_));
    }
    pool_->run(nsub, one);
  } else {
    for (int r = 0; r < nsub; r++) one(r);
  }
  size_t ntu = 0, nlev = 0;
  for (auto &r : job.subs) { if (r.rc < 0) return r.rc; ntu += r.tus.size(); nlev += r.levels.size(); }
  const bool bi = (job.sh.is_b || job.sh.weighted) && job.any_bi.load(std::memory_order_relaxed) != 0;
  const DecInputLayout lay = job.lay = DecInputLayout(pw_, ph_, ctbl_, ntu, nlev, job.b4x.size(), bi);
  if (!grow_job_input(job, lay.upload_bytes())) return DEC_ERR_GPU;
  if (bi) memcpy(job.h_in + lay.x_off, job.b4x.data(), lay.nb4x * sizeof(B4L1));
  DecTu *tus = (DecTu *)(job.h_in + lay.tu_off); uint32_t *lev = (uint32_t *)(job.h_in + lay.lev_off);
  size_t t = 0, l = 0;
  for (int r = 0; r < nsub; r++) {
    SubOut &so = job.subs[(size_t)r];
    const int cy0 = job.geom[(size_t)r].cy0, cy1 = job.geom[(size_t)r].cy1, cx0 = job.geom[(size_t)r].cx0, cx1 = job.geom[(size_t)r].cx1;
    if (t) {
      for (int cy = cy0; cy < cy1; cy++) {
        for (int cx = cx0; cx < cx1; cx++) if (job.ctu[cy * wc + cx].count & 0xffffffu) job.ctu[cy * wc + cx].first += (uint32_t)t;
        if (ctbl_ == 6) for (int ry = 2 * cy; ry < 2 * cy + 2; ry++) for (int rx = 2 * cx0; rx < 2 * cx1; rx++) { TuRange &g = job.region[ry * 2 * wc + rx]; if (g.count) g.first += (uint32_t)t; }
      }
    }
    for (DecTu td : so.tus) { td.offset += (uint32_t)l; tus[t++] = td; }
    if (!so.levels.empty()) memcpy(lev + l, so.levels.data(), so.levels.size() * sizeof(uint32_t));
    l += so.levels.size();
  }
  if (ctbl_ < 6) {
    const int rw = pw_ >> 5, nreg = rw * (ph_ >> 5);
    auto region_of = [&](const DecTu &d) { const int X = d.plane ? d.x * 2 : d.x, Y = d.plane ? d.y * 2 : d.y; return (Y >> 5) * rw + (X >> 5); };
    for (int g = 0; g < nreg; g++) { job.region[g].first = 0; job.region[g].count = 0; }
    for (size_t k = 0; k < ntu; k++) job.region[region_of(tus[k])].count++;
    uint32_t at = 0;
    for (int g = 0; g < nreg; g++) { job.region[g].first = at; at += job.region[g].count; job.region[g].count = 0; }
    uint32_t *idx = (uint32_t *)(job.h_in + lay.i_off);
    for (size_t k = 0; k < ntu; k++) { TuRange &g = job.region[region_of(tus[k])]; idx[g.first + g.count++] = (uint32_t)k; }
  }
  job.ntu = ntu; job.nlev = nlev;
  if (job.scan_gaps) {
    for (int a = 0; a < wc * hc; a++) if (job.miss_map[(size_t)a]) { if (!job.missing.empty() && job.missing.back().first + job.missing.back().second == a) job.missing.back().second++; else job.missing.emplace_back(a, 1); }
    if (!job.missing.empty()) { miss = job.miss_map; job.lf_restricted = true; }
  }
  if (job.lf_restricted) {
    const int n = wc * hc;
    std::vector<int> order((size_t)n, 0), slice((size_t)n, 0);
    {
      int ts = 0, cur = -1; size_t next = 0;
      for (const PicJob::SubGeom &g : job.geom)
        for (int cy = g.cy0; cy < g.cy1; cy++)
          for (int cx = g.cx0; cx < g.cx1; cx++) {
            const int a = cy * wc + cx;
            while (next < job.lf_slices.size() && job.lf_slices[next].first == a) { cur = (int)next; next++; }
            order[(size_t)a] = ts++; slice[(size_t)a] = cur < 0 ? 0 : cur;
          }
      if (next != job.lf_slices.size()) return DEC_ERR_INVALID;
    }
    uint8_t *nb = job.h_in + lay.nb_off;
    const int per = 1 << (ctbl_ - 2), b4w = pw_ / 4;
    for (int cy = 0; cy < hc; cy++)
      for (int cx = 0; cx < wc; cx++) {
        const int c = cy * wc + cx; uint8_t m = 0xff;
        for (int dy = -1; dy <= 1; dy++)
          for (int dx = -1; dx <= 1; dx++) {
            const int nx = cx + dx, ny = cy + dy;
            if ((!dx && !dy) || nx < 0 || ny < 0 || nx >= wc || ny >= hc) continue;
            const int q = ny * wc + nx, later = order[(size_t)q] > order[(size_t)c] ? q : c;
            const bool closed = (job.ctu_tile[c] != job.ctu_tile[q] && !job.pps.across_tiles && job.ctb_cut.empty()) ||
                                (!miss.empty() && (miss[(size_t)c] || miss[(size_t)q])) ||
                                (!job.lf_slices.empty() && slice[(size_t)c] != slice[(size_t)q] && !job.lf_slices[(size_t)slice[(size_t)later]].second);
            const int k = (dy + 1) * 3 + (dx + 1);
            if (closed) m &= (uint8_t)~(1u << (k > 4 ? k - 1 : k));
          }
        nb[c] = m;
        if (!(m & (1u << 3))) for (int k = 0; k < per && (cy * per + k) * 4 < h_; k++) job.b4[(size_t)(cy * per + k) * b4w + cx * per].flags &= (uint8_t)~(B4_EDGE_V | B4_TU_V);
        if (!(m & (1u << 1))) for (int k = 0; k < per && (cx * per + k) * 4 < w_; k++) job.b4[(size_t)(cy * per) * b4w + cx * per + k].flags &= (uint8_t)~(B4_EDGE_H | B4_TU_H);
      }
  }
  return 0;
}

}
```

### kvazzup_amd/csrc/decoder.h

```cpp
#pragma once
#include <hip/hip_runtime.h>
#include <stdint.h>
#include <string.h>
#include <string>
#include <atomic>
#include <condition_variable>
#include <deque>
#include <functional>
#include <map>
#include <memory>
#include <mutex>
#include <thread>
#include <vector>
#include "hevc_core.h"
#include "dec_syntax.h"
#include "host_pool.h"
#include "dec_frame.h"
#include "dec_kernels.h"
#include "batch.h"

namespace kvzx {

enum { PM_INTER = 0, PM_INTRA = 1, PM_SKIP = 2, PM_NONE = 255 };
enum DecKernelId { DK_INTER = 0, DK_INTRA, DK_DEBLOCK, DK_HOST_PARSE, DK_SAO, DK_INTRA_P, DK_COUNT };

struct DecodedPicture {
  int width = 0, height = 0;
  int coded_w = 0, coded_h = 0;
  const uint8_t *host[3] = {nullptr, nullptr, nullptr}; int host_pitch[3] = {0, 0, 0};
  const uint8_t *dev[3] = {nullptr, nullptr, nullptr}; int dev_pitch[3] = {0, 0, 0};
  int poc = 0; int64_t pts = 0; uint32_t fps_num = 0, fps_den = 0; bool is_intra = false;
  int cvs = 0, num_reorder = 0;
  uint64_t serial = 0;
  int missing_ctbs = 0, total_ctbs = 0;
};

struct OwnedPic {
  DecodedPicture pic;
  std::vector<uint8_t> host;
  uint8_t *dev = nullptr;
};

class FrameWorkers {
 public:
  explicit FrameWorkers(int n) { for (int i = 0; i < n; i++) t_.emplace_back([this] { name_this_thread("kvzx-parse"); run(); }); }
  ~FrameWorkers() { { std::lock_guard<std::mutex> l(m_); quit_ = true; } cv_.notify_all(); for (auto &t : t_) t.join(); }
  void submit(std::function<void()> f) { { std::lock_guard<std::mutex> l(m_); q_.push_back(std::move(f)); } cv_.notify_one(); }
 private:
  void run()
  {
    for (;;) {
      std::function<void()> f;
      { std::unique_lock<std::mutex> l(m_); cv_.wait(l, [this] { return quit_ || !q_.empty(); }); if (q_.empty()) return; f = std::move(q_.front()); q_.pop_front(); }
      f();
    }
  }
  std::vector<std::thread> t_; std::mutex m_; std::condition_variable cv_; std::deque<std::function<void()>> q_; bool quit_ = false;
};

struct ColMotion {
  struct Mv { int16_t mv[2][2]; int32_t ref_poc[2]; uint8_t used; uint8_t lt; uint8_t pad[2]; };
  int w16 = 0, h16 = 0, hc = 0, poc = 0;
  std::vector<Mv> mv;
  std::unique_ptr<std::atomic<uint8_t>[]> row_done;
  std::unique_ptr<std::atomic<uint8_t>[]> row_cols;
  int cols = 1;
};

struct ConcealMotion {
  struct E { int16_t mv[2]; int32_t ref_poc; uint8_t lt, none, pad[2]; };
  int w16 = 0, h16 = 0;
  std::vector<E> e;
};

class Decoder {
 public:
  explicit Decoder(int device) : device_(device) {}
  bool set_concealment(int mode) { if ((mode != 2 && mode != 3) || !jobs_.empty() || (mode == 3 && band_nrows_ > 0)) return false; conceal_mode_ = mode; return true; }
  int concealment() const { return conceal_mode_; }
  bool set_partial_pictures(bool on) { if (!jobs_.empty() || (on && band_nrows_ > 0)) return false; partial_ = on; return true; }
  bool partial_pictures() const { return partial_; }
  int damage_log(int32_t *triples, int cap) const { const int n = (int)(damage_log_.size() / 3); for (int i = 0; triples && i < n && i < cap; i++) memcpy(triples + 3 * i, &damage_log_[(size_t)3 * i], 3 * sizeof(int32_t)); return n; }
  void set_frame_threads(int n) { if (jobs_.empty()) frame_threads_ = n < 1 ? 1 : (n > 32 ? 32 : n); }
  int frame_threads() const { return frame_threads_; }
  ~Decoder();
  bool start(std::string *error);
  int decode_nal(const uint8_t *data, size_t len, int64_t pts);
  bool get_picture(DecodedPicture *out);
  void set_download(bool on) { download_ = on; }
  bool set_parse_only() { if (jobs_.empty() && !started_) parse_only_ = true; return parse_only_; }
  struct ProbeStats { uint64_t pictures = 0, tus = 0, levels = 0, digest = 0xcbf29ce484222325ull, bins = 0; double parse_ms = 0; };
  ProbeStats parse_probe_stats() const { return probe_; }
  void set_output_hold(int n) { output_hold_ = n < 1 ? 1 : (n > 8 ? 8 : n); }
  void set_profiling(int every) { profiling_ = every > 0; prof_every_ = every > 0 ? every : 1; }
  void set_parse_threads(int n) { if (!pool_) parse_threads_ = n < 1 ? 1 : n; }
  void get_kernel_times(double *ms, uint64_t *launches, bool reset);
  bool debug_copy(const char *what, void *dst, size_t bytes);
  int last_error() const { return last_error_; }
  void set_check_hash(bool on) { check_hash_ = on; }
  void set_no_cropping(bool on) { no_crop_ = on; }
  void set_max_temporal_id(int t) { max_tid_ = t < 0 ? 0 : (t > 7 ? 7 : t); }
  void hash_stats(int *checked, int *mismatch) const { if (checked) *checked = hash_checked_; if (mismatch) *mismatch = hash_mismatch_; }
  void flush() {}
  int pending() const { return (int)(job_head_ - job_tail_) + (gpu_job_ ? 1 : 0) + (int)gpu_q_.size(); }

  struct alignas(128) SubOut { std::vector<uint32_t> levels; std::vector<DecTu> tus; int rc = 0; };
  struct alignas(64) Progress { std::atomic<int> v{0}; char pad[60]; };
  struct PicJob {
    std::vector<uint8_t> rbsp; size_t data_off = 0, data_len = 0;
    std::vector<size_t> sub_start;
    std::vector<uint8_t> seg_end_row; std::vector<size_t> row_restart;
    struct SubGeom { int cy0, cy1, cx0, cx1, tile_cy0, tile_cy1, tc; };
    std::vector<SubGeom> geom; std::vector<uint8_t> seg_end_sub;
    std::vector<uint8_t> ctb_cut, ctb_slice; std::vector<size_t> ctb_data; std::vector<int8_t> slice_qps; std::vector<uint8_t> ds_saved;
    bool ambiguous_end = false;
    bool lf_restricted = false; std::vector<std::pair<int, uint8_t>> lf_slices;
    struct Undo { int poc = 0, prev_poc = 0; bool is_ref = false, used = false, seen_irap = false; long decode_idx = 0; std::shared_ptr<ColMotion> motion; std::shared_ptr<ConcealMotion> cmotion; std::vector<std::pair<uint64_t, int>> vwait; bool standin = false; } undo;
    SliceHdr sh; std::shared_ptr<const DecSps> sps; DecPps pps;
    int64_t pts = 0; int crop[4] = {0, 0, 0, 0}; uint32_t fps_num = 0, fps_den = 0;
    int slot = 0;
    int cvs = 0;
    uint64_t serial = 0;
    struct Conceal { int first, second; int poc = 0, src_poc = 0; std::shared_ptr<const ConcealMotion> motion; Conceal(int buf, int src) : first(buf), second(src) {} };
    bool scan_gaps = false;
    std::vector<uint8_t> miss_map; std::vector<int> row_seg_start;
    std::vector<std::pair<int, int>> missing; int fill_src = -1, fill_src_poc = 0; std::shared_ptr<const ConcealMotion> fill_motion;
    std::vector<Conceal> conceal;
    bool starts_cvs = false, discard_prior = false;
    int nref = 0; int ref_poc[16]; uint8_t ref_slot[16];
    int nref1 = 0; int ref_poc1[16]; uint8_t ref_slot1[16];
    uint8_t ref_lt[16] = {}, ref_lt1[16] = {};
    bool no_backward = true;
    struct MvF { int16_t mv[2][2]; int8_t ref[2]; };
    std::vector<MvF> mvf; std::vector<B4L1> b4x; std::atomic<int> any_bi{0};
    uint8_t *early_dst = nullptr; std::atomic<int> early_rows{0};
    std::shared_ptr<ColMotion> col, own;
    std::shared_ptr<ConcealMotion> cown;
    uint8_t *h_in = nullptr; size_t h_in_cap = 0; size_t ntu = 0, nlev = 0;
    DecInputLayout lay;
    B4Rec *b4 = nullptr; TuRange *region = nullptr, *ctu = nullptr; uint8_t *ctu_tile = nullptr; SaoParams *sao = nullptr;
    std::vector<uint8_t> pred_mode, ct_depth, intra_mode;
    std::vector<SubOut> subs; std::vector<uint8_t> wpp_saved;
    std::unique_ptr<Progress[]> row_progress; int row_progress_n = 0;
    alignas(64) bool any_intra = false; bool any_inter = false;
    alignas(64) bool across_slices = true;
    std::atomic<int> state{0}; int rc = 0; double parse_ms = 0;
    hipEvent_t done = nullptr;
    std::atomic<int> launched{1};
    std::vector<uint8_t> expect_hash;
    long launch_idx = 0;
    hipEvent_t dl_done = nullptr; int dl_buf = -1;
    struct EvPair { hipEvent_t a, b; int id; }; std::vector<EvPair> ev; size_t ev_used = 0;
    PicJob() {}
    PicJob(const PicJob &) {}
  };
  bool set_band(int row0, int nrows) { if ((conceal_mode_ == 3 || partial_) && nrows > 0) return false; if (jobs_.empty()) { band_row0_ = row0; band_nrows_ = nrows; } return true; }
  size_t band_halo_bytes() const { return (size_t)pw_ * 8; }
  bool band_export(int stage, uint8_t *d_buf);
  bool band_import(int stage, const uint8_t *d_buf);
  bool band_ready() const { return band_nrows_ > 0 && gpu_job_ != nullptr; }
  bool band_deblock();
  int band_finish();
  int pw() const { return pw_; }
  int ph() const { return ph_; }

 private:
  bool ensure_buffers(int w, int h, int ctb_log2);
  void free_buffers();
  int decode_slice(const uint8_t *rbsp, size_t len, int nal_type, int64_t pts);
  size_t unescape(const uint8_t *data, size_t len); int decode_parameter_set(int nal_type, BitReader &r);
  int hash_sei(const uint8_t *rbsp, size_t len);
  int verify_hash(const PicJob &job, const std::vector<uint8_t> &want);
  bool check_hash_ = false; int hash_checked_ = 0, hash_mismatch_ = 0;
  int parse_job(PicJob &job, bool row_parallel);
  int parse_substream(PicJob &job, int sub, const uint8_t *data, size_t len, SubOut &out);
  int close_open_picture();
  int close_free_picture(PicJob &job);
  void take_back_job(PicJob &job); void file_damage(const PicJob &job); std::vector<uint8_t> layout_of(const PicJob &job) const; std::vector<uint8_t> damaged_layout_; uint32_t take_backs_ = 0;
  struct FreeSeg { int address; bool dependent; int slice_qp; std::vector<size_t> subs; };
  struct LfSlice { int address; bool across; };
  struct OpenPicture {
    bool active = false, guessed_one_row = false, free = false, irap = false;
    int subs = 0, rows = 0, pps_id = 0, nal_type = 0;
    bool cur_dependent = false; int cur_qp = 26;
    std::vector<FreeSeg> segs; std::vector<LfSlice> lf;
  } asm_;
  bool free_stream_ = false;
  void note_lf_restrictions(PicJob &job);
  int finish_oldest();
  void drop_pending();
  size_t nctb() const { return (size_t)(pw_ >> ctbl_) * (ph_ >> ctbl_); }
  bool prepare_jobs(int w, int h, int ctb_log2);
  bool grow_job_input(PicJob &job, size_t bytes);
  void bind_job(PicJob &job);
  struct ChainSet; int launch_gpu(PicJob &job);
  int fill_concealed(PicJob &job); int fill_missing(PicJob &job); uint8_t *input_buffer(PicJob &job, int ib);
  DecFrame picture_frame(PicJob &job, const DecInputLayout &lay, const ChainSet &cs, uint8_t *d_in) const;
  bool upload(PicJob &job, const DecInputLayout &lay, uint8_t *d_in, int ib, bool batched);
  int post_to_batcher(PicJob &job, const DecFrame &f, uint8_t *d_in, int ib); int launch_self(PicJob &job, const DecFrame &f, uint8_t *d_in, int ib, bool alt);
  template <class F> bool each_buffer_used(const PicJob &job, F &&visit);
  int complete_gpu(PicJob &job);
  int alloc_slot(); struct DpbPic; bool alloc_picture(DpbPic &p);
  void sync_main();
  bool batch_attached_ = false, batch_used_ = false;

  int device_; bool started_ = false;
  bool parse_only_ = false; ProbeStats probe_; void probe_book(PicJob &job, double ms);
  hipStream_t stream_up_ = nullptr; hipEvent_t up_done_[9] = {};
  hipStream_t stream_ = nullptr, stream_dl_ = nullptr;
  std::shared_ptr<const DecSps> sps_[16]; DecPps pps_[64]; uint32_t vps_fps_num_ = 0, vps_fps_den_ = 0;
  int w_ = 0, h_ = 0, pw_ = 0, ph_ = 0; int ctbl_ = 6;
  std::vector<PicJob> jobs_; int frame_threads_ = 1; long job_head_ = 0, job_tail_ = 0;
  int submit_job(PicJob &job, int nal_type, bool irap);
  int submit_closed(PicJob &job, int rc);
  struct SliceCtx;
  bool slice_front(SliceCtx &c, int &rc);
  void sequence_state(const SliceCtx &c);
  int apply_rps_and_build_lists(SliceCtx &c);
  PicJob &open_job(const SliceCtx &c, const DecPps &pp, int slot);
  int append_segment_tiles(PicJob &job, const SliceCtx &c, int address);
  int append_segment(PicJob &job, const SliceCtx &c, const DecPps &pp, int address);
  std::deque<OwnedPic> ready_q_; OwnedPic cur_owned_;
  struct Waiting { OwnedPic pic; int cvs; };
  std::deque<Waiting> reorder_q_; int cvs_ = 0, reorder_ = 0;
  bool pop_reordered(bool flush);
  static constexpr int kOutHold = 8;
  long nal_calls_ = 0;
  std::deque<std::pair<long, uint8_t *>> retired_out_;
  std::deque<std::pair<long, OwnedPic>> retired_owned_;
  static constexpr size_t kOwnedPoolMax = 24;
  std::vector<std::pair<size_t, uint8_t *>> owned_pool_; std::map<const uint8_t *, size_t> owned_bytes_; hipEvent_t owned_ev_ = nullptr;
  uint8_t *owned_alloc(size_t bytes); void owned_release(uint8_t *p); void owned_free(uint8_t *p); bool stash_current_output();
  void free_retired(bool all);
  int decode_nal_inner(const uint8_t *data, size_t len, int64_t pts);
  bool queue_current_output();
  std::unique_ptr<FrameWorkers> workers_;
  struct DpbPic { uint8_t *plane[3] = {nullptr, nullptr, nullptr}; int poc = 0; bool is_ref = false, used = false, is_lt = false, standin = false;
                  long decode_idx = -1000; std::shared_ptr<ColMotion> motion; std::shared_ptr<ConcealMotion> cmotion;
                  hipEvent_t last_dl = nullptr;
                  hipEvent_t last_use = nullptr; bool last_use_alt = false; };
  DpbPic dpb_[KVZ_DEC_MAX_REFS];
  static constexpr int kMaxGpuDepth = 8;
  int gpu_depth_ = 1; std::deque<PicJob *> gpu_q_;
  uint8_t *d_in_[kMaxGpuDepth + 1] = {}; size_t d_in_cap_[kMaxGpuDepth + 1] = {};
  struct ChainSet { hipStream_t stream = nullptr; uint32_t *progress = nullptr, *edge_col = nullptr; unsigned long long *edge_row = nullptr; int16_t *resid[3] = {nullptr, nullptr, nullptr}; uint8_t *work[3] = {nullptr, nullptr, nullptr}; };
  ChainSet chain_[2]; uint32_t chain_gen_ = 0;
  size_t edge_col_words() const { return nctb() * (size_t)(2 << ctbl_); } size_t edge_row_words() const { return edge_col_words() / 4; }
  bool build_chain(ChainSet &cs, hipStream_t clear_on); void free_chain(ChainSet &cs);
  uint32_t *intra_order_ = nullptr, *err_ = nullptr; uint32_t *h_err_ = nullptr;
  char alt_prio_ = 'n'; long intra_seq_ = 0; bool alt_failed_ = false;
  bool ensure_alt();
  static constexpr int kOutRing = 16;
  uint8_t *h_out_[kOutRing] = {}; size_t h_out_cap_ = 0;
  void describe_output(const PicJob &job, DecodedPicture &o, int buf) const;
  int queue_download(PicJob &job);
  int start_ready_downloads();
  long launched_ = 0; int out_slot_ = 0; int output_hold_ = 2;
  char prio_dl_ = 'n', prio_up_ = 'n';
  char prio_ = 'n';
  int band_row0_ = 0, band_nrows_ = 0; uint8_t *band_din_ = nullptr; DecFrame band_f_{};
  double t_parse_max_ = 0;
  bool spin_wait_ = false;
  PicJob *gpu_job_ = nullptr;
  int prev_poc_ = 0, cur_tid_ = 0; bool seen_irap_ = false;
  int max_tid_ = 7; bool no_crop_ = false;
  bool after_eos_ = false;
  std::vector<std::pair<uint64_t, int>> vwait_; std::vector<uint64_t> discarded_; uint64_t pic_serial_ = 0;
  int conceal_ref(int poc, bool is_lt); std::vector<PicJob::Conceal> pending_conceal_; uint64_t concealed_ = 0;
  int conceal_mode_ = 2;
  static std::vector<int16_t> conceal_displacements(const ConcealMotion *m, int w16, int h16, int p, int s);
  int16_t *d_standin_tab_ = nullptr; size_t standin_tab_cap_ = 0;
  int standin_slot_ = -1; std::vector<int16_t> standin_tab_;
  float standin_ms_ = -1;
  bool partial_ = false; int cur_fill_src_ = -1, avoid_slot_ = -1;
  void choose_fill_source(int poc, bool last_decoded, const std::vector<int> &fresh);
  std::vector<int32_t> damage_log_;
  uint32_t *d_fill_ctbs_ = nullptr; size_t fill_ctbs_cap_ = 0; int16_t *d_fill_tab_ = nullptr; size_t fill_tab_cap_ = 0;
  std::vector<int16_t> fill_tab_;
  bool cur_discard_ = false;
  bool cur_no_rasl_ = false;
  bool skip_rasl_ = false;
  bool download_ = true, profiling_ = false, prof_now_ = false; int prof_every_ = 1;
  bool pic_ready_ = false; DecodedPicture out_;
  int last_error_ = 0;
  double t_nal_ = 0, t_wait_ = 0, t_stage_ = 0, t_api_ = 0, t_sync_ = 0;
  std::vector<uint8_t> rbsp_;
  std::vector<size_t> epb_;
  std::vector<size_t> sub_start_;
  std::unique_ptr<OrderedPool> pool_; int parse_threads_ = 16; std::mutex pool_mutex_;
  PicJob *timed_job_ = nullptr;
  double k_ms_[DK_COUNT] = {0}; uint64_t k_n_[DK_COUNT] = {0};
  template <class F> void timed(int id, F &&launch, hipStream_t st = nullptr);
};

}
```

### kvazzup_amd/csrc/decoder.hip

```cpp
#include <chrono>
#include <cstdio>
#include <cstdlib>
#include <cstring>
#include "stream_pool.h"
#include "pic_hash.h"
#include "decoder.h"
#include "scaling_tables.h"

namespace kvzx {

#define HIP_TRY(expr) do { hipError_t e_ = (expr); if (e_ != hipSuccess) { fprintf(stderr, "kvazzup_amd: %s failed: %s\n", #expr, hipGetErrorString(e_)); return false; } } while (0)

namespace {
struct Tick { std::chrono::steady_clock::time_point t0 = std::chrono::steady_clock::now(); double ms() const { return std::chrono::duration<double, std::milli>(std::chrono::steady_clock::now() - t0).count(); } };
}

void Decoder::drop_pending()
{
  if (gpu_job_ || !gpu_q_.empty()) { sync_main(); if (stream_dl_) hipStreamSynchronize(stream_dl_); }
  if (gpu_job_) { gpu_job_->ev_used = 0; gpu_job_->dl_buf = -1; gpu_job_ = nullptr; }
  for (PicJob *j : gpu_q_) { j->ev_used = 0; j->dl_buf = -1; }
  gpu_q_.clear();
  for (; job_tail_ != job_head_; job_tail_++) {
    PicJob &job = jobs_[(size_t)(job_tail_ % jobs_.size())];
    while (job.state.load(std::memory_order_acquire) != 2) std::this_thread::yield();
    job.state.store(0, std::memory_order_relaxed);
  }
}

void Decoder::sync_main()
{
  if (batch_used_) { DecBatcher::get(device_).drain(this); batch_used_ = false; }
  hipStreamSynchronize(stream_);
  if (chain_[1].stream) hipStreamSynchronize(chain_[1].stream);
}

Decoder::~Decoder()
{
  if (getenv("KVAZZUP_AMD_TRACE")) fprintf(stderr, "kvazzup_amd decoder thread ms: nal %.1f  wait_parse %.1f  stage %.1f  gpu_api %.1f  gpu_sync %.1f  longest parse %.2f  (pictures %ld)\n", t_nal_, t_wait_, t_stage_, t_api_, t_sync_, t_parse_max_, job_tail_);
  if (parse_only_) { for (auto &j : jobs_) free(j.h_in); return; }
  drop_pending();
  workers_.reset();
  if (stream_) sync_main();
  if (batch_attached_) { DecBatcher::get(device_).detach(); batch_attached_ = false; }
  if (h_err_ && *h_err_) fprintf(stderr, "kvazzup_amd: decoder device error flags 0x%x (last picture)\n", *h_err_);
  for (auto &j : jobs_) { for (auto &e : j.ev) { hipEventDestroy(e.a); hipEventDestroy(e.b); } if (j.done) hipEventDestroy(j.done); if (j.dl_done) hipEventDestroy(j.dl_done); }
  free_buffers();
  free_retired(true);
  for (auto &o : ready_q_) owned_free(o.dev);
  for (auto &w : reorder_q_) owned_free(w.pic.dev);
  owned_free(cur_owned_.dev);
  for (auto &b : owned_pool_) owned_free(b.second);
  owned_pool_.clear();
  if (owned_ev_) hipEventDestroy(owned_ev_);
  if (stream_dl_ != stream_up_) stream_release(stream_dl_, device_, 'L', 'l');
  stream_release(stream_up_, device_, 'U', prio_up_);
  for (auto &e : up_done_) if (e) hipEventDestroy(e);
  if (h_err_) hipHostFree(h_err_);
  if (chain_[1].stream) stream_release(chain_[1].stream, device_, 'E', alt_prio_);
  stream_release(stream_, device_, 'D', prio_);
}

bool Decoder::start(std::string *error)
{
  if (parse_only_) { frame_threads_ = 1; started_ = true; return true; }
  int ndev = 0;
  if (hipGetDeviceCount(&ndev) != hipSuccess || ndev <= device_) {
    if (error) *error = "no usable HIP device (this library has no CPU fallback)";
    return false;
  }
  HIP_TRY(hipSetDevice(device_));
  spin_wait_ = getenv("KVAZZUP_AMD_SPIN") != nullptr;
  {
    const char *prio = getenv("KVAZZUP_AMD_PRIO");
    prio_ = (prio && strlen(prio) >= 4) ? prio[3] : 'n';
    HIP_TRY(stream_acquire(&stream_, device_, 'D', prio_));
    chain_[0].stream = stream_;
  }
  {
    const char *prio = getenv("KVAZZUP_AMD_PRIO");
    prio_dl_ = (prio && strlen(prio) >= 5) ? prio[4] : 'n'; prio_up_ = (prio && strlen(prio) >= 6) ? prio[5] : 'n';
  }
  HIP_TRY(stream_acquire(&stream_up_, device_, 'U', prio_up_));
  stream_dl_ = stream_up_;
  if (const char *e = getenv("KVAZZUP_AMD_DL")) if (!strcmp(e, "own")) HIP_TRY(stream_acquire(&stream_dl_, device_, 'L', 'l'));
  for (auto &e : up_done_) HIP_TRY(hipEventCreateWithFlags(&e, hipEventDisableTiming));
  HIP_TRY(hipHostMalloc(&h_err_, sizeof(uint32_t), hipHostMallocMapped));
  *h_err_ = 0;
  { void *dp = nullptr; HIP_TRY(hipHostGetDevicePointer(&dp, h_err_, 0)); err_ = (uint32_t *)dp; }
  DecBatcher::get(device_).attach(stream_); batch_attached_ = true;
  started_ = true;
  return true;
}

void Decoder::free_buffers()
{
  for (auto &j : jobs_) { if (j.h_in) hipHostFree(j.h_in); j.h_in = nullptr; j.h_in_cap = 0; j.col.reset(); j.own.reset(); j.cown.reset(); }
  hipFree(d_standin_tab_); d_standin_tab_ = nullptr; standin_tab_cap_ = 0; standin_slot_ = -1; standin_tab_.clear();
  hipFree(d_fill_ctbs_); d_fill_ctbs_ = nullptr; fill_ctbs_cap_ = 0; hipFree(d_fill_tab_); d_fill_tab_ = nullptr; fill_tab_cap_ = 0; fill_tab_.clear();
  if (stream_dl_) hipStreamSynchronize(stream_dl_);
  for (auto &p : h_out_) { if (p) retired_out_.emplace_back(nal_calls_, p); p = nullptr; }
  for (auto &p : d_in_) { hipFree(p); p = nullptr; } for (auto &c : d_in_cap_) c = 0;
  free_chain(chain_[0]); hipFree(intra_order_); intra_order_ = nullptr;
  if (chain_[1].stream) { hipStreamSynchronize(chain_[1].stream); free_chain(chain_[1]); stream_release(chain_[1].stream, device_, 'E', alt_prio_); chain_[1].stream = nullptr; }
  alt_failed_ = false;
  for (auto &p : dpb_) { hipFree(p.plane[0]); p = DpbPic(); }
  w_ = h_ = pw_ = ph_ = 0;
}

bool Decoder::build_chain(ChainSet &cs, hipStream_t clear_on)
{
  const size_t npx = (size_t)pw_ * ph_;
  auto cleared = [&](void *p, size_t bytes) { return clear_on ? hipMemsetAsync(p, 0, bytes, clear_on) : hipMemset(p, 0, bytes); };
  HIP_TRY(hipMalloc(&cs.progress, sizeof(uint32_t) * (3 * nctb() + 1))); HIP_TRY(cleared(cs.progress, sizeof(uint32_t) * (3 * nctb() + 1)));
  HIP_TRY(hipMalloc(&cs.edge_col, edge_col_words() * sizeof(uint32_t))); HIP_TRY(cleared(cs.edge_col, edge_col_words() * sizeof(uint32_t)));
  HIP_TRY(hipMalloc(&cs.edge_row, edge_row_words() * 8)); HIP_TRY(cleared(cs.edge_row, edge_row_words() * 8));
  for (int c = 0; c < 3; c++) { HIP_TRY(hipMalloc(&cs.resid[c], sizeof(int16_t) * (c ? npx / 4 : npx))); HIP_TRY(hipMalloc(&cs.work[c], c ? npx / 4 : npx)); }
  return true;
}
void Decoder::free_chain(ChainSet &cs)
{
  hipFree(cs.progress); hipFree(cs.edge_col); hipFree(cs.edge_row); for (int c = 0; c < 3; c++) { hipFree(cs.resid[c]); hipFree(cs.work[c]); }
  cs = ChainSet{cs.stream};
}

void Decoder::bind_job(PicJob &job)
{
  uint8_t *p = job.h_in;
  job.b4 = (B4Rec *)p; job.region = (TuRange *)(p + job.lay.region_off); job.ctu = (TuRange *)(p + job.lay.ctu_off);
  job.ctu_tile = p + job.lay.tile_off; job.sao = (SaoParams *)(p + job.lay.sao_off);
}

bool Decoder::grow_job_input(PicJob &job, size_t bytes)
{
  if (bytes <= job.h_in_cap) return true;
  const size_t cap = bytes + bytes / 2;
  uint8_t *p = nullptr;
  if (parse_only_) p = (uint8_t *)aligned_alloc(64, (cap + 63) & ~(size_t)63);
  else if (hipSetDevice(device_) != hipSuccess || hipHostMalloc(&p, cap, hipHostMallocDefault) != hipSuccess) return false;
  if (!p) return false;
  if (job.h_in) {
    memcpy(p, job.h_in, job.lay.fixed_bytes() < job.h_in_cap ? job.lay.fixed_bytes() : job.h_in_cap);
    if (!parse_only_ && job.early_rows.load(std::memory_order_acquire) > 0) hipStreamSynchronize(stream_up_);
    if (parse_only_) free(job.h_in); else hipHostFree(job.h_in);
  }
  job.h_in = p; job.h_in_cap = cap;
  bind_job(job);
  return true;
}

bool Decoder::ensure_buffers(int w, int h, int ctb_log2)
{
  if (w == w_ && h == h_ && ctb_log2 == ctbl_) return true;
  while (!parse_only_ && w_ && (!gpu_q_.empty() || job_tail_ != job_head_)) {
    const int rc = finish_oldest();
    if (rc < 0 || (rc > 0 && pic_ready_ && !stash_current_output())) { drop_pending(); break; }
  }
  while (!parse_only_ && w_ && pop_reordered(true)) {}
  if (parse_only_) {
    for (auto &j : jobs_) { free(j.h_in); j.h_in = nullptr; j.h_in_cap = 0; }
    if (jobs_.empty()) jobs_ = std::vector<PicJob>(3);
    gpu_depth_ = 1;
    if (!prepare_jobs(w, h, ctb_log2)) return false;
    for (auto &d : dpb_) { d = DpbPic(); d.plane[0] = (uint8_t *)(uintptr_t)64; }
    seen_irap_ = false;
    return true;
  }
  drop_pending();
  sync_main();
  free_buffers();
  if (jobs_.empty()) {
    const char *e = getenv("KVAZZUP_AMD_DEC_GPU_DEPTH");
    gpu_depth_ = e ? atoi(e) : (frame_threads_ >= 4 ? (frame_threads_ >= 24 ? 8 : (frame_threads_ >= 12 ? 4 : 3)) : 1);
    if (gpu_depth_ > kMaxGpuDepth) gpu_depth_ = kMaxGpuDepth;
    if (gpu_depth_ > frame_threads_ - 1) gpu_depth_ = frame_threads_ - 1;
    if (gpu_depth_ < 1 || band_nrows_ > 0) gpu_depth_ = 1;
    jobs_ = std::vector<PicJob>((size_t)frame_threads_ + 2);
  }
  if (!prepare_jobs(w, h, ctb_log2)) return false;
  h_out_cap_ = (size_t)pw_ * ph_ * 3 / 2;
  for (int i = 0; i <= gpu_depth_; i++) { d_in_cap_[i] = jobs_[0].lay.fixed_bytes() + (1 << 20); HIP_TRY(hipMalloc(&d_in_[i], d_in_cap_[i])); }
  if (!build_chain(chain_[0], nullptr)) return false; chain_gen_ = 0;
  {
    const int wc = ctbs_in(w_, ctbl_), hc = ctbs_in(h_, ctbl_);
    std::vector<uint32_t> order;
    const int r0 = band_nrows_ > 0 ? band_row0_ : 0, nr = band_nrows_ > 0 ? band_nrows_ : hc;
    if (r0 < 0 || r0 + nr > hc) return false;
    for (int d = 0; d < wc + 2 * nr; d++) for (int cy = 0; cy < nr; cy++) { const int cx = d - 2 * cy; if (cx >= 0 && cx < wc) order.push_back((uint32_t)((r0 + cy) * wc + cx)); }
    HIP_TRY(hipMalloc(&intra_order_, sizeof(uint32_t) * order.size()));
    HIP_TRY(hipMemcpy(intra_order_, order.data(), sizeof(uint32_t) * order.size(), hipMemcpyHostToDevice));
  }
  for (int s = 0; s < 6; s++) if (!alloc_picture(dpb_[s])) return false;
  seen_irap_ = false;
  HIP_TRY(hipDeviceSynchronize());
  return true;
}

int Decoder::conceal_ref(int poc, bool is_lt)
{
  const int s = alloc_slot();
  if (s < 0) return -1;
  DpbPic &d = dpb_[s];
  d.poc = poc; d.is_ref = true; d.used = true; d.is_lt = is_lt; d.standin = true; d.motion.reset(); d.cmotion.reset();
  pending_conceal_.emplace_back(s, -2);
  if (concealed_++ < 3) fprintf(stderr, "kvazzup_amd: decoder: reference picture with POC %d never arrived -- the nearest reference picture (or a grey one) stands in\n", poc);
  return s;
}

bool Decoder::alloc_picture(DpbPic &p)
{
  const size_t npx = (size_t)pw_ * ph_;
  if (hipMalloc(&p.plane[0], npx * 3 / 2) != hipSuccess) { p.plane[0] = nullptr; return false; }
  p.plane[1] = p.plane[0] + npx; p.plane[2] = p.plane[1] + npx / 4;
  HIP_TRY(hipMemset(p.plane[0], 128, npx * 3 / 2));
  return true;
}
bool Decoder::prepare_jobs(int w, int h, int ctb_log2)
{
  w_ = w; h_ = h; pw_ = (w + 63) & ~63; ph_ = (h + 63) & ~63; ctbl_ = ctb_log2;
  const size_t nb4 = (size_t)pw_ * ph_ / 16;
  for (auto &j : jobs_) {
    j.lay = DecInputLayout(pw_, ph_, ctbl_, 0, 0, 0, false);
    if (!grow_job_input(j, j.lay.fixed_bytes() + (1 << 16))) return false;
    memset(j.h_in, 0, j.lay.fixed_bytes());
    j.pred_mode.assign(nb4 / 4, PM_NONE); j.ct_depth.assign(nb4 / 4, 0); j.intra_mode.assign(nb4, 1);
  }
  return true;
}

int Decoder::alloc_slot()
{
  for (int s = 0; s < KVZ_DEC_MAX_REFS; s++) {
    DpbPic &p = dpb_[s];
    if (p.is_ref || s == avoid_slot_ || job_head_ - p.decode_idx <= output_hold_ + (gpu_depth_ - 1)) continue;
    if (!p.plane[0] && parse_only_) p.plane[0] = (uint8_t *)(uintptr_t)64;
    if (!p.plane[0]) { if (hipSetDevice(device_) != hipSuccess || !alloc_picture(p)) return -1; hipDeviceSynchronize(); }
    return s;
  }
  return -1;
}

template <class F> void Decoder::timed(int id, F &&launch, hipStream_t st)
{
  if (!prof_now_) { launch(); return; }
  if (!st) st = stream_;
  PicJob &j = *timed_job_;
  if (j.ev_used == j.ev.size()) { PicJob::EvPair p; hipEventCreate(&p.a); hipEventCreate(&p.b); p.id = id; j.ev.push_back(p); }
  PicJob::EvPair &p = j.ev[j.ev_used++]; p.id = id;
  hipEventRecord(p.a, st); launch(); hipEventRecord(p.b, st);
}
bool Decoder::ensure_alt()
{
  if (chain_[1].stream) return true;
  if (alt_failed_) return false;
  if (hipSetDevice(device_) != hipSuccess) return false;
  { const char *e = getenv("KVAZZUP_AMD_DEC_ALT_PRIO"); alt_prio_ = e ? e[0] : 'l'; }
  ChainSet cs;
  auto build = [&]() -> bool { HIP_TRY(stream_acquire(&cs.stream, device_, 'E', alt_prio_)); return build_chain(cs, cs.stream); };
  if (!build()) {
    if (cs.stream) hipStreamSynchronize(cs.stream);
    free_chain(cs); stream_release(cs.stream, device_, 'E', alt_prio_); (void)hipGetLastError();
    alt_failed_ = true; return false;
  }
  chain_[1] = cs;
  return true;
}
void Decoder::get_kernel_times(double *ms, uint64_t *launches, bool reset)
{
  for (int i = 0; i < DK_COUNT; i++) { if (ms) ms[i] = k_ms_[i]; if (launches) launches[i] = k_n_[i]; }
  if (reset) for (int i = 0; i < DK_COUNT; i++) { k_ms_[i] = 0; k_n_[i] = 0; }
}

void Decoder::free_retired(bool all)
{
  while (!retired_out_.empty() && (all || nal_calls_ - retired_out_.front().first > kOutHold)) { hipHostFree(retired_out_.front().second); retired_out_.pop_front(); }
  while (!retired_owned_.empty() && (all || nal_calls_ - retired_owned_.front().first > kOutHold)) { if (all) owned_free(retired_owned_.front().second.dev); else owned_release(retired_owned_.front().second.dev); retired_owned_.pop_front(); }
}

int Decoder::decode_nal(const uint8_t *data, size_t len, int64_t pts)
{
  nal_calls_++;
  if (!retired_out_.empty() || !retired_owned_.empty()) free_retired(false);
  const int rc = decode_nal_inner(data, len, pts);
  if (rc >= 0 && ((pic_ready_ && out_.num_reorder > 0) || !reorder_q_.empty())) {
    if (pic_ready_ && out_.num_reorder == 0) {
      while (pop_reordered(true)) {}
      if (!queue_current_output()) return last_error_ = DEC_ERR_GPU;
    } else if (pic_ready_) {
      const int cvs = out_.cvs; reorder_ = out_.num_reorder;
      if (!queue_current_output()) return last_error_ = DEC_ERR_GPU;
      reorder_q_.push_back(Waiting{std::move(ready_q_.back()), cvs}); ready_q_.pop_back();
    }
    const bool eos = len >= 2 && [&] { size_t i = 0; while (i + 2 < len && data[i] == 0) i++; const uint8_t *q = (i >= 2 && i < len && data[i] == 1) ? data + i + 1 : data; const int t = (q[0] >> 1) & 0x3f; return t == 36 || t == 37; }();
    if (ready_q_.empty() && !pop_reordered(eos && pending() == 0)) return 0;
  } else {
  if (ready_q_.empty()) return rc;
  if (rc < 0) return rc;
  if (pic_ready_ && !queue_current_output()) return last_error_ = DEC_ERR_GPU;
  }
  if (cur_owned_.dev || !cur_owned_.host.empty()) retired_owned_.emplace_back(nal_calls_, std::move(cur_owned_));
  cur_owned_ = OwnedPic();
  cur_owned_ = std::move(ready_q_.front());
  ready_q_.pop_front();
  out_ = cur_owned_.pic;
  size_t off = 0;
  for (int c = 0; c < 3; c++) {
    const int h = c ? out_.height / 2 : out_.height;
    if (!cur_owned_.host.empty()) { out_.host[c] = cur_owned_.host.data() + off; off += (size_t)out_.host_pitch[c] * h; }
  }
  pic_ready_ = true;
  return 1;
}

bool Decoder::pop_reordered(bool flush)
{
  if (reorder_q_.empty()) return false;
  int first_cvs = reorder_q_.front().cvs, n = 0; size_t best = 0;
  for (const Waiting &w : reorder_q_) if (w.cvs < first_cvs) first_cvs = w.cvs;
  bool later = false;
  for (size_t i = 0; i < reorder_q_.size(); i++) {
    const Waiting &w = reorder_q_[i];
    if (w.cvs != first_cvs) { later = true; continue; }
    if (n++ == 0 || w.pic.pic.poc < reorder_q_[best].pic.pic.poc) best = i;
  }
  if (!(flush || later || n > reorder_)) return false;
  ready_q_.push_back(std::move(reorder_q_[best].pic));
  reorder_q_.erase(reorder_q_.begin() + (long)best);
  return true;
}

uint8_t *Decoder::owned_alloc(size_t bytes)
{
  for (size_t i = 0; i < owned_pool_.size(); i++) if (owned_pool_[i].first == bytes) { uint8_t *p = owned_pool_[i].second; owned_pool_.erase(owned_pool_.begin() + (long)i); return p; }
  for (auto &b : owned_pool_) owned_free(b.second);
  owned_pool_.clear();
  uint8_t *p = nullptr;
  if (hipSetDevice(device_) != hipSuccess || hipMalloc(&p, bytes) != hipSuccess) return nullptr;
  owned_bytes_[p] = bytes;
  return p;
}
void Decoder::owned_release(uint8_t *p)
{
  if (!p) return;
  auto it = owned_bytes_.find(p);
  if (it != owned_bytes_.end() && owned_pool_.size() < kOwnedPoolMax && (owned_pool_.empty() || owned_pool_.front().first == it->second)) { owned_pool_.emplace_back(it->second, p); return; }
  owned_free(p);
}
void Decoder::owned_free(uint8_t *p)
{
  if (!p) return;
  owned_bytes_.erase(p);
  hipFree(p);
}
bool Decoder::queue_current_output()
{
  OwnedPic o;
  o.pic = out_;
  if (download_) {
    for (int c = 0; c < 3; c++) {
      const uint8_t *p = out_.host[c];
      o.host.insert(o.host.end(), p, p + (size_t)out_.host_pitch[c] * (c ? out_.height / 2 : out_.height));
    }
  }
  {
    const size_t ny = (size_t)out_.width * out_.height;
    o.dev = owned_alloc(ny * 3 / 2);
    if (!o.dev) return false;
// ... 764 lines not shown
      if (frame_threads_ > 1 && !spin_wait_)
        return nap_until([&] { hipError_t r = hipEventQuery(ev); return r == hipSuccess ? 1 : (r == hipErrorNotReady ? 0 : -1); });
      return hipEventSynchronize(ev) == hipSuccess;
    };
    if (download_ && job.dl_buf < 0) {
      if (!wait(job.done)) return DEC_ERR_GPU;
      const int rc = queue_download(job); if (rc < 0) return rc;
    }
    if (!wait(download_ ? job.dl_done : job.done)) return DEC_ERR_GPU;
    t_sync_ += tk.ms();
  }
  if (*h_err_) { fprintf(stderr, "kvazzup_amd: decoder device error flags 0x%x\n", *h_err_); return DEC_ERR_GPU; }
  if (!job.expect_hash.empty() && job.missing.empty()) {
    const std::vector<uint8_t> want = std::move(job.expect_hash); job.expect_hash.clear();
    const int rc = verify_hash(job, want);
    if (rc < 0) last_error_ = rc;
  }
  if (job.ev_used) {
    for (size_t i = 0; i < job.ev_used; i++) { float ms = 0; hipEventElapsedTime(&ms, job.ev[i].a, job.ev[i].b); k_ms_[job.ev[i].id] += ms; k_n_[job.ev[i].id]++; }
    job.ev_used = 0;
  }
  if (job.sh.no_output) { job.dl_buf = -1; return 0; }
  if (!discarded_.empty() && std::find(discarded_.begin(), discarded_.end(), job.serial) != discarded_.end()) { job.dl_buf = -1; return 0; }
  describe_output(job, out_, download_ ? job.dl_buf : -1);
  out_slot_ = job.slot;
  job.dl_buf = -1;
  pic_ready_ = true;
  return 1;
}

std::vector<int16_t> Decoder::conceal_displacements(const ConcealMotion *m, int w16, int h16, int p, int s)
{
  std::vector<int16_t> tab((size_t)w16 * h16 * 4, 0);
  if (!m || m->w16 != w16 || m->h16 != h16) return tab;
  auto clip3 = [](long long lo, long long hi, long long v) { return (int)(v < lo ? lo : (v > hi ? hi : v)); };
  std::vector<int> v((size_t)w16 * h16 * 2, 0);
  const int tb = clip3(-128, 127, (long long)p - s);
  for (size_t b = 0; b < (size_t)w16 * h16; b++) {
    const ConcealMotion::E &e = m->e[b];
    const int td = clip3(-128, 127, (long long)s - e.ref_poc);
    if (e.none || e.lt || td == 0) continue;
    const int tx = (16384 + (abs(td) >> 1)) / td, f = clip3(-4096, 4095, (tb * tx + 32) >> 6);
    for (int k = 0; k < 2; k++) { const int q = f * e.mv[k], a = (abs(q) + 127) >> 8; v[2 * b + k] = clip3(-32768, 32767, q < 0 ? -a : a); }
  }
  for (int y = 0; y < h16; y++)
    for (int x = 0; x < w16; x++) {
      const size_t b = (size_t)y * w16 + x;
      const int vx = v[2 * b], vy = v[2 * b + 1];
      int agree = 0;
      auto near = [&](int nx, int ny) { if (nx < 0 || ny < 0 || nx >= w16 || ny >= h16) return; const size_t n = (size_t)ny * w16 + nx; agree += abs(v[2 * n] - vx) <= 4 && abs(v[2 * n + 1] - vy) <= 4; };
      near(x - 1, y); near(x + 1, y); near(x, y - 1); near(x, y + 1);
      if (agree < 2) continue;
      tab[4 * b] = (int16_t)((vx + 2) >> 2); tab[4 * b + 1] = (int16_t)((vy + 2) >> 2); tab[4 * b + 2] = (int16_t)((vx + 4) >> 3); tab[4 * b + 3] = (int16_t)((vy + 4) >> 3);
    }
  return tab;
}

int Decoder::fill_concealed(PicJob &job)
{
  const size_t npx = (size_t)pw_ * ph_;
  for (PicJob *j : gpu_q_) while (!j->launched.load(std::memory_order_acquire)) futex_wait(j->launched, 0);
  if (hipDeviceSynchronize() != hipSuccess) return DEC_ERR_GPU;
  hipEvent_t ev[2] = {nullptr, nullptr};
  auto stamp = [&](int k, hipStream_t st) { if (profiling_ && (ev[k] || hipEventCreate(&ev[k]) == hipSuccess)) hipEventRecord(ev[k], st); };
  auto elapsed = [&] { float ms = 0; if (profiling_ && ev[0] && ev[1] && hipEventSynchronize(ev[1]) == hipSuccess && hipEventElapsedTime(&ms, ev[0], ev[1]) == hipSuccess) standin_ms_ = ms; };
  for (const auto &c : job.conceal) {
    uint8_t *dst = dpb_[c.first].plane[0], *src = c.second >= 0 ? dpb_[c.second].plane[0] : nullptr;
    if (conceal_mode_ == 3 && dst) {
      const int w16 = (w_ + 15) / 16, h16 = (h_ + 15) / 16;
      const bool moved = src && src != dst;
      standin_slot_ = c.first;
      standin_tab_ = moved ? conceal_displacements(c.motion.get(), w16, h16, c.poc, c.src_poc) : std::vector<int16_t>((size_t)w16 * h16 * 4, 0);
      if (moved) {
        const size_t bytes = standin_tab_.size() * sizeof(int16_t);
        if (bytes > standin_tab_cap_) { hipFree(d_standin_tab_); standin_tab_cap_ = 0; if (hipMalloc(&d_standin_tab_, bytes) != hipSuccess) { d_standin_tab_ = nullptr; return DEC_ERR_GPU; } standin_tab_cap_ = bytes; }
        if (hipMemcpy(d_standin_tab_, standin_tab_.data(), bytes, hipMemcpyHostToDevice) != hipSuccess) return DEC_ERR_GPU;
        stamp(0, stream_);
        launch_dec_standin(dpb_[c.first].plane, dpb_[c.second].plane, d_standin_tab_, w_, h_, pw_, stream_);
        stamp(1, stream_);
        if (hipGetLastError() != hipSuccess || hipStreamSynchronize(stream_) != hipSuccess) return DEC_ERR_GPU;
        elapsed();
        continue;
      }
    }
    stamp(0, nullptr);
    if (dst && (src && src != dst ? hipMemcpy(dst, src, npx * 3 / 2, hipMemcpyDeviceToDevice) : hipMemset(dst, 128, npx * 3 / 2)) != hipSuccess) return DEC_ERR_GPU;
    stamp(1, nullptr); elapsed();
  }
  if (hipDeviceSynchronize() != hipSuccess) return DEC_ERR_GPU;
  for (hipEvent_t e : ev) if (e) hipEventDestroy(e);
  job.conceal.clear(); return 0;
}
void Decoder::choose_fill_source(int poc, bool last_decoded, const std::vector<int> &fresh)
{
  int best = -1;
  for (int q = 0; q < KVZ_DEC_MAX_REFS; q++) {
    if (!dpb_[q].is_ref || !dpb_[q].used || std::find(fresh.begin(), fresh.end(), q) != fresh.end()) continue;
    if (last_decoded) { if (!dpb_[q].standin && (best < 0 || dpb_[q].decode_idx > dpb_[best].decode_idx)) best = q; continue; }
    const long long dq = llabs((long long)dpb_[q].poc - poc), db = best < 0 ? 0 : llabs((long long)dpb_[best].poc - poc);
    if (best < 0 || dq < db || (dq == db && dpb_[q].poc < dpb_[best].poc)) best = q;
  }
  cur_fill_src_ = avoid_slot_ = best;
}
int Decoder::fill_missing(PicJob &job)
{
  while (!job.launched.load(std::memory_order_acquire)) futex_wait(job.launched, 0);
  if (hipDeviceSynchronize() != hipSuccess) return DEC_ERR_GPU;
  const int wc = ctbs_in(w_, ctbl_), total = wc * ctbs_in(h_, ctbl_);
  std::vector<uint32_t> list;
  for (const auto &m : job.missing) for (int k = 0; k < m.second; k++) if (m.first + k >= 0 && m.first + k < total) list.push_back((uint32_t)(m.first + k));
  if (list.empty()) return 0;
  if (list.size() * sizeof(uint32_t) > fill_ctbs_cap_) { hipFree(d_fill_ctbs_); fill_ctbs_cap_ = 0; if (hipMalloc(&d_fill_ctbs_, (size_t)total * sizeof(uint32_t)) != hipSuccess) { d_fill_ctbs_ = nullptr; return DEC_ERR_GPU; } fill_ctbs_cap_ = (size_t)total * sizeof(uint32_t); }
  if (hipMemcpy(d_fill_ctbs_, list.data(), list.size() * sizeof(uint32_t), hipMemcpyHostToDevice) != hipSuccess) return DEC_ERR_GPU;
  uint8_t *const *dst = dpb_[job.slot].plane;
  uint8_t *const *src = job.fill_src >= 0 && job.fill_src != job.slot && dpb_[job.fill_src].plane[0] ? dpb_[job.fill_src].plane : nullptr;
  const int16_t *d_tab = nullptr;
  const int w16 = (w_ + 15) / 16, h16 = (h_ + 15) / 16;
  fill_tab_.assign((size_t)w16 * h16 * 4, 0);
  if (conceal_mode_ == 3 && src) {
    fill_tab_ = conceal_displacements(job.fill_motion.get(), w16, h16, job.sh.poc, job.fill_src_poc);
    const size_t bytes = fill_tab_.size() * sizeof(int16_t);
    if (bytes > fill_tab_cap_) { hipFree(d_fill_tab_); fill_tab_cap_ = 0; if (hipMalloc(&d_fill_tab_, bytes) != hipSuccess) { d_fill_tab_ = nullptr; return DEC_ERR_GPU; } fill_tab_cap_ = bytes; }
    if (hipMemcpy(d_fill_tab_, fill_tab_.data(), bytes, hipMemcpyHostToDevice) != hipSuccess) return DEC_ERR_GPU;
    d_tab = d_fill_tab_;
  }
  hipEvent_t ev[2] = {nullptr, nullptr};
  if (profiling_) for (auto &e : ev) if (hipEventCreate(&e) != hipSuccess) e = nullptr;
  if (ev[0]) hipEventRecord(ev[0], stream_);
  launch_dec_fill_ctbs(dst, src, d_tab, d_fill_ctbs_, (int)list.size(), ctbl_, w_, h_, pw_, stream_);
  if (ev[1]) hipEventRecord(ev[1], stream_);
  if (hipGetLastError() != hipSuccess || hipStreamSynchronize(stream_) != hipSuccess) return DEC_ERR_GPU;
  if (ev[0] && ev[1]) { float ms = 0; if (hipEventElapsedTime(&ms, ev[0], ev[1]) == hipSuccess) standin_ms_ = ms; }
  for (hipEvent_t e : ev) if (e) hipEventDestroy(e);
  return 0;
}
uint8_t *Decoder::input_buffer(PicJob &job, int ib)
{
  const size_t bytes = job.lay.upload_bytes();
  if (bytes > d_in_cap_[ib]) {
    if (job.early_dst) { hipStreamSynchronize(stream_up_); job.early_dst = nullptr; }
    hipFree(d_in_[ib]); d_in_cap_[ib] = bytes + bytes / 2;
    if (hipMalloc(&d_in_[ib], d_in_cap_[ib]) != hipSuccess) { d_in_[ib] = nullptr; d_in_cap_[ib] = 0; }
  }
  return d_in_[ib];
}
DecFrame Decoder::picture_frame(PicJob &job, const DecInputLayout &lay, const ChainSet &cs, uint8_t *d_in) const
{
  DecFrame f; memset(&f, 0, sizeof(f));
  f.w = w_; f.h = h_; f.pw = pw_; f.ph = ph_; f.wc = (w_ + 63) / 64; f.hc = (h_ + 63) / 64;
  f.ctb_log2 = ctbl_; f.cwc = (w_ + (1 << ctbl_) - 1) >> ctbl_; f.chc = (h_ + (1 << ctbl_) - 1) >> ctbl_;
  f.tu_index = lay.indexed ? (const uint32_t *)(d_in + lay.i_off) : nullptr;
  f.b4 = (const B4Rec *)d_in; f.b4x = lay.bi ? (const B4L1 *)(d_in + lay.x_off) : nullptr; f.region = (const TuRange *)(d_in + lay.region_off); f.ctu = (const TuRange *)(d_in + lay.ctu_off);
  f.ctu_tile = d_in + lay.tile_off; f.tus = (const DecTu *)(d_in + lay.tu_off); f.lev = (const uint32_t *)(d_in + lay.lev_off); f.ntu = (int)lay.ntu;
  const bool sao = job.sh.sao_luma || job.sh.sao_chroma;
  for (int c = 0; c < 3; c++) { f.resid[c] = cs.resid[c]; f.rec[c] = sao ? cs.work[c] : dpb_[job.slot].plane[c]; f.out[c] = dpb_[job.slot].plane[c]; }
  for (int k = 0; k < KVZ_DEC_MAX_REFS; k++) for (int c = 0; c < 3; c++) f.ref[k][c] = dpb_[k].plane[c];
  f.sao = sao ? (const SaoParams *)(d_in + lay.sao_off) : nullptr; f.ctu_nb = job.lf_restricted ? d_in + lay.nb_off : nullptr;
  { f.progress = cs.progress; f.intra_order = intra_order_; f.err = err_; const size_t nctu = (size_t)f.cwc * f.chc, S = (size_t)1 << ctbl_;
    f.edge_col[0] = cs.edge_col; f.edge_col[1] = cs.edge_col + nctu * S; f.edge_col[2] = cs.edge_col + nctu * (S + S / 2);
    f.edge_row[0] = cs.edge_row; f.edge_row[1] = cs.edge_row + nctu * (S / 4); f.edge_row[2] = cs.edge_row + nctu * (S / 4 + S / 8); }
  if (job.any_intra) f.chain_gen = chain_gen_;
  f.cb_qp_offset = (int8_t)job.pps.cb_qp_offset; f.cr_qp_offset = (int8_t)job.pps.cr_qp_offset; f.beta_offset = (int8_t)(2 * job.sh.beta_offset_div2); f.tc_offset = (int8_t)(2 * job.sh.tc_offset_div2);
  f.intra_direct = job.any_inter ? 1 : 0;
  f.strong_intra = (uint8_t)job.sps->strong_intra; f.tiles = job.pps.tile_rows > 1 || job.pps.tile_cols > 1 || job.slice_qps.size() > 1 || !job.missing.empty();
  f.general = (uint8_t)(job.pps.tile_rows > 1 || job.pps.tile_cols > 1 || job.slice_qps.size() > 1 || !job.missing.empty() || job.sps->pcm_depth[0] != 0);
  f.cip = (uint8_t)(job.pps.cip && job.any_inter);
  f.tq_bypass = (uint8_t)(job.pps.tq_bypass || (job.sps->pcm_depth[0] && job.sps->pcm_no_filter));
  const std::vector<uint8_t> *sc = !job.sps->scaling ? nullptr : (job.pps.scaling ? job.pps.scaling.get() : job.sps->scaling.get());
  if (sc) { memcpy(job.h_in + lay.scaling_off, sc->data(), KVZ_SCALING_BYTES); f.scaling = d_in + lay.scaling_off; }
  if (job.sh.weighted && lay.bi) { memcpy(job.h_in + lay.wt_off, job.sh.wt, sizeof(job.sh.wt)); f.wt = (const DecWt *)(d_in + lay.wt_off); f.wt_log2[0] = job.sh.wt_log2[0]; f.wt_log2[1] = job.sh.wt_log2[1]; }
  if (band_nrows_ > 0) { f.row0 = band_row0_; f.nrows = band_nrows_; }
  return f;
}
bool Decoder::upload(PicJob &job, const DecInputLayout &lay, uint8_t *d_in, int ib, bool batched)
{
  const size_t up_from = (!batched && job.early_dst && job.early_dst == d_in && job.early_rows.load(std::memory_order_acquire) == ctbs_in(h_, ctbl_)) ? lay.region_off : 0;
  job.early_dst = nullptr;
  if (hipMemcpyAsync(d_in + up_from, job.h_in + up_from, lay.upload_bytes() - up_from, hipMemcpyHostToDevice, stream_up_) != hipSuccess) return false;
  return hipEventRecord(up_done_[ib], stream_up_) == hipSuccess;
}
int Decoder::post_to_batcher(PicJob &job, const DecFrame &f, uint8_t *d_in, int ib)
{
  DecBatchItem it; it.f = f; it.d_f = (const DecFrame *)(d_in + job.lay.frame_off);
  it.inter = job.any_inter; it.intra = job.any_intra; it.deblock = !job.sh.deblock_disabled; it.sao = job.sh.sao_luma || job.sh.sao_chroma;
  it.wait0 = up_done_[ib]; it.wait1 = dpb_[job.slot].last_dl; dpb_[job.slot].last_dl = nullptr;
  it.done = job.done; it.launched = &job.launched; it.owner = this; it.profile = prof_now_;
  job.launched.store(0, std::memory_order_relaxed);
  DecBatcher::get(device_).submit(it); batch_used_ = true;
  return 0;
}
template <class F> bool Decoder::each_buffer_used(const PicJob &job, F &&visit)
{
  bool ok = visit(dpb_[job.slot]);
  for (int k = 0; ok && k < job.nref; k++) ok = visit(dpb_[job.ref_slot[k]]);
  for (int k = 0; ok && k < job.nref1; k++) ok = visit(dpb_[job.ref_slot1[k]]);
  return ok;
}
int Decoder::launch_self(PicJob &job, const DecFrame &f, uint8_t *d_in, int ib, bool alt)
{
  const hipStream_t st = chain_[alt].stream;
  if (hipStreamWaitEvent(st, up_done_[ib], 0) != hipSuccess) return DEC_ERR_GPU;
  if (dpb_[job.slot].last_dl) { if (hipStreamWaitEvent(st, dpb_[job.slot].last_dl, 0) != hipSuccess) return DEC_ERR_GPU; dpb_[job.slot].last_dl = nullptr; }
  if (chain_[1].stream && !each_buffer_used(job, [&](DpbPic &d) { return !(d.last_use && d.last_use_alt != alt) || hipStreamWaitEvent(st, d.last_use, 0) == hipSuccess; })) return DEC_ERR_GPU;
  if (job.any_inter) timed(DK_INTER, [&] { launch_dec_inter(f, st); }, st);
  if (job.any_intra) timed(job.any_inter ? DK_INTRA_P : DK_INTRA, [&] { launch_dec_intra_resid(f, st); launch_dec_intra(f, st); }, st);
  if (band_nrows_ > 0) { band_f_ = f; band_din_ = d_in; }
  else if (!job.sh.deblock_disabled) timed(DK_DEBLOCK, [&] { launch_dec_deblock(f, st); }, st);
  if (f.sao) timed(DK_SAO, [&] { launch_dec_sao(f, st); }, st);
  if (hipEventRecord(job.done, st) != hipSuccess) return DEC_ERR_GPU;
  each_buffer_used(job, [&](DpbPic &d) { d.last_use = job.done; d.last_use_alt = alt; return true; });
  return 0;
}
int Decoder::launch_gpu(PicJob &job)
{
  if (hipSetDevice(device_) != hipSuccess) return DEC_ERR_GPU;
  if (!job.conceal.empty()) { const int rc = fill_concealed(job); if (rc < 0) return rc; }
  prof_now_ = profiling_ && (launched_ % prof_every_) == 0; timed_job_ = &job; job.ev_used = 0;
  if (!job.done && hipEventCreateWithFlags(&job.done, hipEventDisableTiming) != hipSuccess) return DEC_ERR_GPU;
  Tick tk_api; const int ib = (int)(launched_ % (gpu_depth_ + 1));
  uint8_t *const d_in = input_buffer(job, ib); if (!d_in) return DEC_ERR_GPU;
  DecBatcher &batcher = DecBatcher::get(device_);
  const bool batched = band_nrows_ == 0 && batch_attached_ && batcher.active() && !(job.pps.cip && job.any_inter && job.any_intra);
  static const bool alt_off = getenv("KVAZZUP_AMD_DEC_ONE_CHAIN") != nullptr;
  bool alt = !alt_off && !batched && band_nrows_ == 0 && frame_threads_ > 1 && gpu_depth_ > 1 && job.any_intra && !job.any_inter && ((intra_seq_++) & 1);
  if (alt && !ensure_alt()) alt = false;
  if (job.any_intra && ++chain_gen_ >= (1u << 24)) {
    sync_main();
    for (const ChainSet &c : chain_) if (c.stream && (hipMemsetAsync(c.edge_col, 0, edge_col_words() * sizeof(uint32_t), c.stream) != hipSuccess || hipMemsetAsync(c.edge_row, 0, edge_row_words() * 8, c.stream) != hipSuccess)) return DEC_ERR_GPU;
    chain_gen_ = 1;
  }
  if (band_nrows_ > 0) {
    bool ok = !(job.sh.sao_luma || job.sh.sao_chroma) && !job.sps->tmvp && job.pps.tile_cols == 1 && frame_threads_ == 1, top = false, bottom = false;
    for (int t = 0; t <= job.pps.tile_rows; t++) { top |= job.pps.row_bd[t] == band_row0_; bottom |= job.pps.row_bd[t] == band_row0_ + band_nrows_; }
    if (!ok || !top || !bottom) return DEC_ERR_UNSUPPORTED;
  }
  const DecFrame f = picture_frame(job, job.lay, chain_[alt], d_in);
  if (!batched && batch_used_) { batcher.drain(this); batch_used_ = false; }
  if (batched && chain_[1].stream) hipStreamSynchronize(chain_[1].stream);
  if (batched) memcpy(job.h_in + job.lay.frame_off, &f, sizeof(f));
  if (!upload(job, job.lay, d_in, ib, batched)) return DEC_ERR_GPU;
  job.dl_buf = -1; job.launch_idx = launched_;
  if (const int rc = batched ? post_to_batcher(job, f, d_in, ib) : launch_self(job, f, d_in, ib, alt); rc < 0) return rc;
  if (!job.missing.empty()) { const int rc = fill_missing(job); if (rc < 0) return rc; }
  t_api_ += tk_api.ms(); launched_++;
  if (band_nrows_ > 0) gpu_job_ = &job; else gpu_q_.push_back(&job);
  return 0;
}

bool Decoder::band_export(int stage, uint8_t *d_buf)
{
  if (band_nrows_ <= 0 || !gpu_job_ || !d_buf) return false;
  PicJob &job = *gpu_job_;
  const int y = stage == 0 ? (band_row0_ + band_nrows_) * 64 - 4 : band_row0_ * 64 - 4;
  if (y < 0 || y + 4 > ph_) return false;
  size_t o = 0;
  if (hipMemcpyAsync(d_buf + o, dpb_[job.slot].plane[0] + (size_t)y * pw_, (size_t)pw_ * 4, hipMemcpyDeviceToDevice, stream_) != hipSuccess) return false;
  o += (size_t)pw_ * 4;
  for (int c = 1; c < 3; c++) { if (hipMemcpyAsync(d_buf + o, dpb_[job.slot].plane[c] + (size_t)(y / 2) * (pw_ / 2), (size_t)pw_, hipMemcpyDeviceToDevice, stream_) != hipSuccess) return false; o += (size_t)pw_; }
  if (stage == 0 && hipMemcpyAsync(d_buf + o, band_din_ + (size_t)(y / 4) * (pw_ / 4) * sizeof(B4Rec), (size_t)(pw_ / 4) * sizeof(B4Rec), hipMemcpyDeviceToDevice, stream_) != hipSuccess) return false;
  return hipStreamSynchronize(stream_) == hipSuccess;
}
bool Decoder::band_import(int stage, const uint8_t *d_buf)
{
  if (band_nrows_ <= 0 || !gpu_job_ || !d_buf) return false;
  PicJob &job = *gpu_job_;
  const int y = stage == 0 ? band_row0_ * 64 - 4 : (band_row0_ + band_nrows_) * 64 - 4;
  if (y < 0 || y + 4 > ph_) return false;
  size_t o = 0;
  if (hipMemcpyAsync(dpb_[job.slot].plane[0] + (size_t)y * pw_, d_buf + o, (size_t)pw_ * 4, hipMemcpyDeviceToDevice, stream_) != hipSuccess) return false;
  o += (size_t)pw_ * 4;
  for (int c = 1; c < 3; c++) { if (hipMemcpyAsync(dpb_[job.slot].plane[c] + (size_t)(y / 2) * (pw_ / 2), d_buf + o, (size_t)pw_, hipMemcpyDeviceToDevice, stream_) != hipSuccess) return false; o += (size_t)pw_; }
  if (stage == 0 && hipMemcpyAsync(band_din_ + (size_t)(y / 4) * (pw_ / 4) * sizeof(B4Rec), d_buf + o, (size_t)(pw_ / 4) * sizeof(B4Rec), hipMemcpyDeviceToDevice, stream_) != hipSuccess) return false;
  return hipStreamSynchronize(stream_) == hipSuccess;
}
bool Decoder::band_deblock()
{
  if (band_nrows_ <= 0 || !gpu_job_) return false;
  if (!gpu_job_->sh.deblock_disabled) launch_dec_deblock(band_f_, stream_);
  return hipEventRecord(gpu_job_->done, stream_) == hipSuccess;
}
int Decoder::band_finish()
{
  if (band_nrows_ <= 0 || !gpu_job_) return 0;
  PicJob *j = gpu_job_; gpu_job_ = nullptr;
  if (hipEventRecord(j->done, stream_) != hipSuccess) return DEC_ERR_GPU;
  return complete_gpu(*j);
}

bool Decoder::get_picture(DecodedPicture *out)
{
  if (!pic_ready_) return false;
  *out = out_;
  return true;
}

bool Decoder::debug_copy(const char *what, void *dst, size_t bytes)
{
  if (!w_) return false;
  const size_t npx = (size_t)pw_ * ph_;
  std::string w(what);
  if (w == "standin") { if (standin_slot_ < 0 || bytes > npx * 3 / 2) return false; return hipDeviceSynchronize() == hipSuccess && hipMemcpy(dst, dpb_[standin_slot_].plane[0], bytes, hipMemcpyDeviceToHost) == hipSuccess; }
  if (w == "standin_ms") { if (bytes != sizeof(float) || standin_ms_ < 0) return false; memcpy(dst, &standin_ms_, sizeof(float)); return true; }
  if (w == "take_backs") { if (bytes != sizeof(uint32_t)) return false; memcpy(dst, &take_backs_, sizeof(uint32_t)); return true; }
  if (w == "fill_mv") { if (fill_tab_.empty() || bytes > fill_tab_.size() * sizeof(int16_t)) return false; memcpy(dst, fill_tab_.data(), bytes); return true; }
  if (w == "partial_layout") {
    std::vector<uint8_t> lay = damaged_layout_;
    if (lay.empty()) {
      if (job_head_ < 1) return false;
      const PicJob &job = jobs_[(size_t)((job_head_ - 1) % (long)jobs_.size())];
      if (job.state.load(std::memory_order_acquire) == 1 || !job.h_in) return false;
      lay = layout_of(job);
    }
    if (bytes != lay.size()) return false;
    memcpy(dst, lay.data(), bytes);
    return true;
  }
  if (w == "standin_mv") { if (standin_slot_ < 0 || bytes > standin_tab_.size() * sizeof(int16_t)) return false; memcpy(dst, standin_tab_.data(), bytes); return true; }
  for (int c = 0; c < 3; c++) {
    size_t n = c ? npx / 4 : npx;
    if (w == std::string("rec") + char('0' + c)) { if (bytes > n) return false; return hipMemcpy(dst, dpb_[out_slot_].plane[c], bytes, hipMemcpyDeviceToHost) == hipSuccess; }
  }
  return false;
}

}
```

Baseline: 9366.

## Add specialized plain-picture CABAC parser path and raw output buffers

Templates the slice parser and residual parser on a PLAIN flag. The flag is chosen per picture when the stream uses a single tile, 64x64 CTBs, P/I slices only, no weighting, no PCM, no transform skip, no QP delta and no collocated MVs, and the specialization compiles those checks away. It also replaces std::vector outputs with a realloc-based RawRun buffer that reserves room once per residual instead of resizing per subblock. When parsing is sequential, all rows write into one shared output, so the later merge becomes two memcpys. This adds code duplication and a second parser path whose correctness depends on the eligibility test.

Measured after the change: 9240. 0.987x the previous value.

```diff
diff --git a/kvazzup_amd/csrc/dec_parse.hip b/kvazzup_amd/csrc/dec_parse.hip
--- a/kvazzup_amd/csrc/dec_parse.hip
+++ b/kvazzup_amd/csrc/dec_parse.hip
@@ -157,13 +157,15 @@
   return g;
 }
 
-__attribute__((always_inline)) inline bool parse_residual_regs(CabacRegs &c, int log2, int cidx, int scan_idx, bool sign_hiding, bool ts_enabled, int *tskip, std::vector<uint32_t> &out)
+template <bool PLAIN>
+__attribute__((always_inline)) inline int parse_residual_regs(CabacRegs &c, int log2, int cidx, int scan_idx, bool sign_hiding, bool ts_enabled, int *tskip, uint32_t *const out)
 {
+  uint32_t *dst = out;
   const ScanTabs &S = scan_tabs();
   const int n = 1 << log2, sbl = log2 - 2, nsb = 1 << sbl;
   const uint8_t *SX = S.x[scan_idx][sbl], *SY = S.y[scan_idx][sbl], *PX = S.x[scan_idx][2], *PY = S.y[scan_idx][2];
   uint8_t csbf[8][8]; memset(csbf, 0, sizeof(csbf));
-  *tskip = (ts_enabled && log2 == 2) ? c.bin(CTX_TS_FLAG + (cidx ? 1 : 0)) : 0;
+  *tskip = (!PLAIN && ts_enabled && log2 == 2) ? c.bin(CTX_TS_FLAG + (cidx ? 1 : 0)) : 0;
   int pre[2];
   for (int d = 0; d < 2; d++) {
     int off, sh, mx = (log2 << 1) - 1, v = 0;
@@ -175,7 +177,7 @@
   if (lx > 3) { int nb = (lx >> 1) - 1; lx = (1 << nb) * (2 + (lx & 1)) + (int)c.bypass_bits(nb); }
   if (ly > 3) { int nb = (ly >> 1) - 1; ly = (1 << nb) * (2 + (ly & 1)) + (int)c.bypass_bits(nb); }
   if (scan_idx == 2) { int tt = lx; lx = ly; ly = tt; }
-  if (lx >= n || ly >= n) return false;
+  if (lx >= n || ly >= n) return -1;
   const int last_sb = S.inv[scan_idx][sbl][((ly >> 2) << sbl) | (lx >> 2)], last_pos = S.inv[scan_idx][2][((ly & 3) << 2) | (lx & 3)];
   int c1 = 1;
   for (int i = last_sb; i >= 0; i--) {
@@ -220,7 +222,7 @@
       if (lev[j] == base) {
         int prefix = 0;
         while (prefix < 32 && c.bypass()) prefix++;
-        if (prefix - 3 + rice > 16) return false;
+        if (prefix - 3 + rice > 16) return -1;
         int rem = prefix <= 3 ? (prefix << rice) + (int)c.bypass_bits(rice)
                               : (((1 << (prefix - 3)) + 3 - 1) << rice) + (int)c.bypass_bits(prefix - 3 + rice);
         lev[j] = base + rem;
@@ -229,34 +231,38 @@
       sum += lev[j];
     }
     if (hidden && (sum & 1)) signs |= 1u;
-    const size_t o0 = out.size();
-    out.resize(o0 + (size_t)nsig);
-    uint32_t *dst = out.data() + o0;
     for (int j = 0; j < nsig; j++) {
       const int v = ((signs >> (nsig - 1 - j)) & 1) ? -lev[j] : lev[j];
       const int xp = PX[pos[j]], yp = PY[pos[j]];
       dst[j] = (uint32_t)((((ys << 2) + yp) * n + (xs << 2) + xp) << 16) | ((uint32_t)clip3(-32768, 32767, v) & 0xffffu);
     }
-    if (c.overrun()) return false;
-  }
-  return !c.overrun();
+    dst += nsig;
+    if (c.overrun()) return -1;
+  }
+  return c.overrun() ? -1 : (int)(dst - out);
 }
 
-bool parse_residual(CabacDec &cd, int log2, int cidx, int scan_idx, bool sign_hiding, bool ts_enabled, int *tskip, std::vector<uint32_t> &out)
+template <bool PLAIN>
+__attribute__((noinline)) bool parse_residual(CabacDec &cd, int log2, int cidx, int scan_idx, bool sign_hiding, bool ts_enabled, int *tskip, Decoder::RawRun<uint32_t> &out)
 {
+  if (!out.room((size_t)1 << (2 * log2))) return false;
   CabacRegs c = cd;
-  const bool ok = parse_residual_regs(c, log2, cidx, scan_idx, sign_hiding, ts_enabled, tskip, out);
+  const int got = parse_residual_regs<PLAIN>(c, log2, cidx, scan_idx, sign_hiding, ts_enabled, tskip, out.base + out.n);
   static_cast<CabacRegs &>(cd) = c;
-  return ok;
+  if (got < 0) return false;
+  out.n += (size_t)got;
+  return true;
 }
 
 struct MvCand { int mvx, mvy, ref_idx; };
 
+template <bool PLAIN>
 struct SliceParser {
   Decoder::PicJob &job; Decoder::SubOut &out;
   const DecSps &sps; const DecPps &pps; const SliceHdr &sh;
   CabacDec c;
-  const int w, h, b4w, b8w, ctbl, mincb, wc, hc;
+  struct CtbLog2 { int v; inline operator int() const { return PLAIN ? 6 : v; } };
+  const int w, h, b4w, b8w; const CtbLog2 ctbl; const int mincb, wc, hc;
   B4Rec *b4; uint8_t *pm, *ctd, *im;
   int ref_y0 = -(1 << 30), ref_y1 = 1 << 30;
   int tile_y0 = 0, tile_y1 = 1 << 30, tile_x0 = 0, tile_x1 = 1 << 30;
@@ -268,7 +274,7 @@
   uint32_t ctu_intra_mask = 0;
 
   SliceParser(Decoder::PicJob &j, Decoder::SubOut &o, int pw)
-      : job(j), out(o), sps(*j.sps), pps(j.pps), sh(j.sh), w(j.sps->width), h(j.sps->height), b4w(pw / 4), b8w(pw / 8), ctbl(j.sps->ctb_log2), mincb(j.sps->min_cb_log2), wc(j.sps->wc()),
+      : job(j), out(o), sps(*j.sps), pps(j.pps), sh(j.sh), w(j.sps->width), h(j.sps->height), b4w(pw / 4), b8w(pw / 8), ctbl{j.sps->ctb_log2}, mincb(j.sps->min_cb_log2), wc(j.sps->wc()),
         hc(j.sps->hc()), b4(j.b4), pm(j.pred_mode.data()), ctd(j.ct_depth.data()), im(j.intra_mode.data())
   { log2_qg = ctbl - pps.qp_delta_depth; }
 
@@ -276,8 +282,10 @@
   inline int b8(int x, int y) const { return (y >> 3) * b8w + (x >> 3); }
   inline bool avail(int, int, int xn, int yn) const
   {
+    if (PLAIN) return xn >= 0 && yn >= 0 && xn < w && yn < h && pm[b8(xn, yn)] != PM_NONE;
     return xn >= tile_x0 && yn >= tile_y0 && xn < w && yn < h && yn < tile_y1 && xn < tile_x1 && pm[b8(xn, yn)] != PM_NONE && (!slice_of || slice_of[(yn >> ctbl) * wc + (xn >> ctbl)] == cur_slice);
   }
+  inline int bypass_cu() const { return PLAIN ? 0 : cu_bypass; }
   void fill_cu8(uint8_t *arr, int x0, int y0, int n, int v)
   {
     const int cols = imin(n, w - x0) >> 3;
@@ -310,12 +318,13 @@
   void emit_tu(const DecTu &td)
   {
     const int X = td.plane ? td.x * 2 : td.x, Y = td.plane ? td.y * 2 : td.y;
+    if (!out.tus.room(1)) { err = DEC_ERR_INVALID; return; }
     if (ctbl == 6) {
       TuRange &r = job.region[(Y >> 5) * (b4w >> 3) + (X >> 5)];
-      if (!r.count) r.first = (uint32_t)out.tus.size();
+      if (!r.count) r.first = (uint32_t)out.tus.n;
       r.count++;
     }
-    out.tus.push_back(td);
+    out.tus.base[out.tus.n++] = td;
   }
 
   bool pb_avail(int xcb, int ycb, int ncbs, int xpb, int ypb, int npbw, int npbh, int part_idx, int xn, int yn) const
@@ -342,6 +351,7 @@
   }
   bool temporal_mv(int xpb, int ypb, int npbw, int npbh, int X, int ref_idx, int &mvx, int &mvy)
   {
+    if (PLAIN) return false;
     ColMotion *col = job.col.get();
     if (!col) return false;
     const int cy = ypb >> ctbl;
@@ -621,7 +631,7 @@
 
   void prediction_unit(int xcb, int ycb, int ncbs, int xp, int yp, int bw, int bh, int part_idx, bool skip, int *merge_out)
   {
-    if (sh.is_b) { prediction_unit_b(xcb, ycb, ncbs, xp, yp, bw, bh, part_idx, skip, merge_out); return; }
+    if (!PLAIN && sh.is_b) { prediction_unit_b(xcb, ycb, ncbs, xp, yp, bw, bh, part_idx, skip, merge_out); return; }
     const int merge = skip ? 1 : c.bin(CTX_MERGE_FLAG);
     if (merge_out) *merge_out = merge;
     int mvx, mvy, ref_idx = 0;
@@ -647,15 +657,15 @@
       mvx = (int16_t)(uint16_t)(cand[mvp][0] + dx); mvy = (int16_t)(uint16_t)(cand[mvp][1] + dy);
     }
     if (ref_idx < 0 || ref_idx >= job.nref) { err = DEC_ERR_INVALID; ref_idx = 0; }
-    if (ref_y1 != (1 << 30) || ref_y0 != -(1 << 30)) {
+    if (!PLAIN && (ref_y1 != (1 << 30) || ref_y0 != -(1 << 30))) {
       const int fy = mvy & 3, fc = mvy & 7;
       const int top = imin(yp + (mvy >> 2) - (fy ? 3 : 0), 2 * ((yp >> 1) + (mvy >> 3) - (fc ? 1 : 0)));
       const int bot = imax(yp + bh + (mvy >> 2) + (fy ? 4 : 0), 2 * ((yp >> 1) + (bh >> 1) + (mvy >> 3) + (fc ? 2 : 0)));
       if (top < ref_y0 || bot > ref_y1) err = DEC_ERR_UNSUPPORTED;
     }
-    B4Rec r; r.mvx = (int16_t)mvx; r.mvy = (int16_t)mvy; r.ref_idx = (int8_t)ref_idx; r.flags = (uint8_t)((cu_bypass ? B4_BYPASS : 0) | ((sh.weighted && ((sh.wt_explicit >> ref_idx) & 1)) ? B4_WT : 0)); r.qp_y = (int8_t)qp_y; r.slot = job.ref_slot[ref_idx];
+    B4Rec r; r.mvx = (int16_t)mvx; r.mvy = (int16_t)mvy; r.ref_idx = (int8_t)ref_idx; r.flags = (uint8_t)((bypass_cu() ? B4_BYPASS : 0) | ((!PLAIN && sh.weighted && ((sh.wt_explicit >> ref_idx) & 1)) ? B4_WT : 0)); r.qp_y = (int8_t)qp_y; r.slot = job.ref_slot[ref_idx];
     fill_recs(xp, yp, bw, bh, r, bw == ncbs && bh == ncbs);
-    if (r.flags & B4_WT) {
+    if (!PLAIN && (r.flags & B4_WT)) {
       B4L1 x; x.mvx = 0; x.mvy = 0; x.slot = 0; x.pad[0] = (uint8_t)ref_idx; x.pad[1] = x.pad[2] = 0;
       const int cols = imin(bw, w - xp) >> 2;
       for (int y = yp; y < yp + bh && y < h; y += 4) { const int i0 = bi(xp, y); for (int i = 0; i < cols; i++) job.b4x[(size_t)(i0 + i)] = x; }
@@ -673,7 +683,7 @@
     const bool chroma_here = log2 > 2, chroma_parent = log2 == 2 && blk == 3;
     const int ccb = chroma_here ? cbf_cb : (chroma_parent ? cbf_cb_parent : 0), ccr = chroma_here ? cbf_cr : (chroma_parent ? cbf_cr_parent : 0);
     const bool cbf_chroma_any = log2 > 2 ? (cbf_cb || cbf_cr) : (cbf_cb_parent || cbf_cr_parent);
-    if ((cbf_luma || cbf_chroma_any) && pps.cu_qp_delta && !qp_delta_coded) {
+    if (!PLAIN && (cbf_luma || cbf_chroma_any) && pps.cu_qp_delta && !qp_delta_coded) {
       int v = 0;
       while (v < 5 && c.bin(CTX_CU_QP_DELTA + (v ? 1 : 0))) v++;
       if (v == 5) { int k = 0; while (k < 16 && c.bypass()) { v += 1 << k; k++; } if (k >= 16) { err = DEC_ERR_INVALID; return; } v += (int)c.bypass_bits(k); }
@@ -687,12 +697,12 @@
     const int lmode = intra ? im[bi(x0, y0)] : 0;
     if (intra || cbf_luma) {
       td.x = (uint16_t)x0; td.y = (uint16_t)y0; td.plane = 0; td.log2 = (uint8_t)log2; td.mode = (uint8_t)lmode; td.qp = (int8_t)qp_y;
-      td.flags = (uint8_t)((intra ? TU_INTRA : 0) | ((intra && log2 == 2) ? TU_DST : 0) | (cu_bypass ? TU_BYPASS : 0));
-      td.offset = (uint32_t)out.levels.size(); td.count = 0;
+      td.flags = (uint8_t)((intra ? TU_INTRA : 0) | ((intra && log2 == 2) ? TU_DST : 0) | (bypass_cu() ? TU_BYPASS : 0));
+      td.offset = (uint32_t)out.levels.n; td.count = 0;
       if (cbf_luma) {
         int ts;
-        if (!parse_residual(c, log2, 0, intra_scan_idx(intra, log2, 0, lmode), pps.sign_hiding != 0 && !cu_bypass, pps.tskip != 0 && !cu_bypass, &ts, out.levels)) { err = DEC_ERR_INVALID; return; }
-        td.count = (uint16_t)(out.levels.size() - td.offset);
+        if (!parse_residual<PLAIN>(c, log2, 0, intra_scan_idx(intra, log2, 0, lmode), pps.sign_hiding != 0 && !bypass_cu(), pps.tskip != 0 && !bypass_cu(), &ts, out.levels)) { err = DEC_ERR_INVALID; return; }
+        td.count = (uint16_t)(out.levels.n - td.offset);
         if (ts) td.flags |= TU_TSKIP;
         for (int y = y0; y < y0 + n && y < h; y += 4) for (int x = x0; x < x0 + n && x < w; x += 4) b4[bi(x, y)].flags |= B4_NZ;
       }
@@ -706,12 +716,12 @@
         if (!intra && !cbf) continue;
         td.x = (uint16_t)cx; td.y = (uint16_t)cy; td.plane = (uint8_t)ci; td.log2 = (uint8_t)clog2; td.mode = (uint8_t)chroma_mode;
         td.qp = (int8_t)kChromaQp[clip3(0, 57, qp_y + (ci == 1 ? sh.cb_qp_offset : sh.cr_qp_offset))];
-        td.flags = (uint8_t)((intra ? TU_INTRA : 0) | (cu_bypass ? TU_BYPASS : 0));
-        td.offset = (uint32_t)out.levels.size(); td.count = 0;
+        td.flags = (uint8_t)((intra ? TU_INTRA : 0) | (bypass_cu() ? TU_BYPASS : 0));
+        td.offset = (uint32_t)out.levels.n; td.count = 0;
         if (cbf) {
           int ts;
-          if (!parse_residual(c, clog2, ci, intra_scan_idx(intra, clog2, ci, chroma_mode), pps.sign_hiding != 0 && !cu_bypass, pps.tskip != 0 && !cu_bypass, &ts, out.levels)) { err = DEC_ERR_INVALID; return; }
-          td.count = (uint16_t)(out.levels.size() - td.offset);
+          if (!parse_residual<PLAIN>(c, clog2, ci, intra_scan_idx(intra, clog2, ci, chroma_mode), pps.sign_hiding != 0 && !bypass_cu(), pps.tskip != 0 && !bypass_cu(), &ts, out.levels)) { err = DEC_ERR_INVALID; return; }
+          td.count = (uint16_t)(out.levels.n - td.offset);
           if (ts) td.flags |= TU_TSKIP;
         }
         emit_tu(td);
@@ -759,7 +769,7 @@
   {
     const int n = 1 << log2cb;
     int skip = 0;
-    cu_bypass = pps.tq_bypass ? c.bin(CTX_TQ_BYPASS) : 0;
+    cu_bypass = (!PLAIN && pps.tq_bypass) ? c.bin(CTX_TQ_BYPASS) : 0;
     if (!sh.is_intra) {
       const int l = avail(x0, y0, x0 - 1, y0) && pm[b8(x0 - 1, y0)] == PM_SKIP, a = avail(x0, y0, x0, y0 - 1) && pm[b8(x0, y0 - 1)] == PM_SKIP;
       skip = c.bin(CTX_SKIP + l + a);
@@ -793,7 +803,7 @@
         }
       }
       fill_cu8(pm, x0, y0, n, cu_pred_mode);
-      if (cu_pred_mode == PM_INTRA && part_mode == PART_2Nx2N && sps.pcm_depth[0] && log2cb >= sps.pcm_min_log2 && log2cb <= sps.pcm_max_log2 && c.terminate()) {
+      if (!PLAIN && cu_pred_mode == PM_INTRA && part_mode == PART_2Nx2N && sps.pcm_depth[0] && log2cb >= sps.pcm_min_log2 && log2cb <= sps.pcm_max_log2 && c.terminate()) {
         const uint8_t *q = c.buf + c.bytes_consumed();
         const size_t need = ((size_t)n * n * sps.pcm_depth[0] + (size_t)n * n / 2 * sps.pcm_depth[1]) / 8;
         if (q > c.end || need > (size_t)(c.end - q)) { err = DEC_ERR_INVALID; return; }
@@ -801,10 +811,11 @@
         for (int ci = 0; ci < 3; ci++) {
           const int shp = ci ? 1 : 0, m = n >> shp, depth = sps.pcm_depth[ci ? 1 : 0];
           DecTu td; td.pad = 0; td.x = (uint16_t)(x0 >> shp); td.y = (uint16_t)(y0 >> shp); td.plane = (uint8_t)ci; td.log2 = (uint8_t)(log2cb - shp); td.mode = 35; td.qp = 0;
-          td.flags = (uint8_t)(TU_INTRA | TU_BYPASS); td.offset = (uint32_t)out.levels.size();
+          td.flags = (uint8_t)(TU_INTRA | TU_BYPASS); td.offset = (uint32_t)out.levels.n;
+          if (!out.levels.room((size_t)m * m)) { err = DEC_ERR_INVALID; return; }
           for (int y = 0; y < m; y++)
-            for (int x = 0; x < m; x++) { const uint32_t v = pr.get(depth) << (8 - depth); if (v) out.levels.push_back((uint32_t)((y * m + x) << 16) | v); }
-          td.count = (uint16_t)(out.levels.size() - td.offset);
+            for (int x = 0; x < m; x++) { const uint32_t v = pr.get(depth) << (8 - depth); if (v) out.levels.base[out.levels.n++] = (uint32_t)((y * m + x) << 16) | v; }
+          td.count = (uint16_t)(out.levels.n - td.offset);
           emit_tu(td);
           ctu_intra_mask |= 1u << ci;
         }
@@ -852,7 +863,7 @@
         static const int cm[4] = {0, 26, 10, 1};
         if (icpm == 4) chroma_mode = intra_modes[0];
         else { chroma_mode = cm[icpm]; if (chroma_mode == intra_modes[0]) chroma_mode = 34; }
-        B4Rec r; r.mvx = 0; r.mvy = 0; r.ref_idx = -1; r.flags = (uint8_t)(cu_bypass ? B4_BYPASS : 0); r.qp_y = (int8_t)qp_y; r.slot = 0;
+        B4Rec r; r.mvx = 0; r.mvy = 0; r.ref_idx = -1; r.flags = (uint8_t)(bypass_cu() ? B4_BYPASS : 0); r.qp_y = (int8_t)qp_y; r.slot = 0;
         fill_recs(x0, y0, n, n, r, true);
         if (!job.any_intra) job.any_intra = true;
       } else {
@@ -885,7 +896,7 @@
       max_trafo_depth = cu_pred_mode == PM_INTRA ? sps.th_depth_intra + (intra_split ? 1 : 0) : sps.th_depth_inter;
       transform_tree(x0, y0, x0, y0, log2cb, 0, 0, 0, 0);
     }
-    if (qp_y != qp_before)
+    if (!PLAIN && qp_y != qp_before)
       for (int y = y0; y < y0 + n && y < h; y += 4) for (int x = x0; x < x0 + n && x < w; x += 4) b4[bi(x, y)].qp_y = (int8_t)qp_y;
     last_qp_y = qp_y;
   }
@@ -899,7 +910,7 @@
       const int l = avail(x0, y0, x0 - 1, y0) && ctd[b8(x0 - 1, y0)] > depth, a = avail(x0, y0, x0, y0 - 1) && ctd[b8(x0, y0 - 1)] > depth;
       split = c.bin(CTX_SPLIT_CU + l + a);
     } else split = log2cb > mincb;
-    if (pps.cu_qp_delta && log2cb >= log2_qg) {
+    if (!PLAIN && pps.cu_qp_delta && log2cb >= log2_qg) {
       qp_delta_coded = false; cu_qp_delta_val = 0;
       int qa = last_qp_y, qb = last_qp_y;
       if (avail(x0, y0, x0 - 1, y0) && ((x0 - 1) >> ctbl) == (x0 >> ctbl)) qa = b4[bi(x0 - 1, y0)].qp_y;
@@ -918,9 +929,20 @@
 
 }
 
-int Decoder::parse_substream(PicJob &job, int sub, const uint8_t *data, size_t len, SubOut &out)
+bool Decoder::plain_picture(const PicJob &job) const
 {
-  SliceParser sp(job, out, pw_);
+  const DecSps &sps = *job.sps; const DecPps &pps = job.pps; const SliceHdr &sh = job.sh;
+  return !force_general_ && pps.tile_cols == 1 && pps.tile_rows == 1 && job.ctb_cut.empty() && ctbl_ == 6 && sps.ctb_log2 == 6 && !sh.is_b && !sh.weighted && !pps.weighted_pred && !pps.weighted_bipred && !pps.tq_bypass && !sps.pcm_depth[0] && !pps.tskip &&
+         !pps.cu_qp_delta && band_nrows_ <= 0 && !job.scan_gaps && job.missing.empty() && !job.lf_restricted && !job.col;
+}
+int Decoder::parse_substream(PicJob &job, int sub, const uint8_t *data, size_t len, SubOut &out, bool sequential)
+{
+  return job.plain ? parse_substream_as<true>(job, sub, data, len, out, sequential) : parse_substream_as<false>(job, sub, data, len, out, sequential);
+}
+template <bool PLAIN>
+int Decoder::parse_substream_as(PicJob &job, int sub, const uint8_t *data, size_t len, SubOut &out, bool sequential)
+{
+  SliceParser<PLAIN> sp(job, out, pw_);
   tl("row0", sub);
   struct RowEnd { int s; ~RowEnd() { tl("row1", s); } } row_end_{sub};
   if (job.sh.is_b) sp.mvf = job.mvf.data();
@@ -931,9 +953,12 @@
   const int first_cy = g.cy0, ncy = g.cy1 - g.cy0, cx0 = g.cx0, cx1 = g.cx1, tw = cx1 - cx0, cols = pps.tile_cols;
   auto tile_starts_at = [&](int cy) { return cy == g.tile_cy0; };
   auto tile_ends_at = [&](int cy) { return cy + 1 == g.tile_cy1; };
+  const bool above_failed = sequential && wpp && !tile_starts_at(first_cy) && job.row_progress[(size_t)(first_cy - 1) * cols + g.tc].v.load(std::memory_order_relaxed) >= (1 << 29);
   int seen_above = 0;
   auto wait_above = [&](int cy, int need) {
+    if (sequential && !above_failed) return true;
     if (!wpp || tile_starts_at(cy)) return true;
+    if (sequential) return false;
     if (need > tw) need = tw;
     if (seen_above < need) {
       std::atomic<int> &p = job.row_progress[(size_t)(cy - 1) * cols + g.tc].v;
@@ -946,8 +971,8 @@
   };
   const int init_type = sh.is_intra ? 0 : (sh.is_b ? (sh.cabac_init_flag ? 1 : 2) : (sh.cabac_init_flag ? 2 : 1));
   CabacDec &c = sp.c;
-  const bool free_slices = !job.ctb_cut.empty();
-  const bool scan = job.scan_gaps && cols == 1 && (!wpp || free_slices);
+  const bool free_slices = !PLAIN && !job.ctb_cut.empty();
+  const bool scan = !PLAIN && job.scan_gaps && cols == 1 && (!wpp || free_slices);
   bool skipping = false;
   size_t first_off = 0;
   if (scan && free_slices) {
@@ -964,6 +989,7 @@
     }
     if (wpp && !skipping) { first_off = job.sub_start[(size_t)first_cy]; if (first_off == SIZE_MAX || first_off >= len) return DEC_ERR_INVALID; }
   }
+  const uint32_t sub_tu0 = (uint32_t)out.tus.n;
   c.start(data + first_off, len - first_off);
   sp.slice_qp = sh.slice_qp;
   if (free_slices) { sp.slice_of = job.ctb_slice.data(); sp.cur_slice = job.ctb_slice[(size_t)first_cy * wc + cx0]; sp.slice_qp = job.slice_qps[(size_t)sp.cur_slice]; }
@@ -994,7 +1020,7 @@
     job.ctu_tile[ctu] = 255; if (free_slices) job.ctb_slice[(size_t)ctu] = 255;
     memset(&job.sao[ctu], 0, sizeof(SaoParams));
     job.miss_map[(size_t)ctu] = 1;
-    if (wpp) job.row_progress[(size_t)(ctu / wc) * cols + g.tc].v.store(ctu % wc - cx0 + 1, std::memory_order_release);
+    if (wpp && !sequential) job.row_progress[(size_t)(ctu / wc) * cols + g.tc].v.store(ctu % wc - cx0 + 1, std::memory_order_release);
   };
   for (int cy = first_cy; cy < first_cy + ncy; cy++) {
     if (cy > first_cy && job.row_restart[(size_t)cy] != SIZE_MAX) {
@@ -1022,7 +1048,7 @@
           sp.last_qp_y = sp.slice_qp;
         }
       }
-      const uint32_t tu0 = (uint32_t)out.tus.size();
+      const uint32_t tu0 = (uint32_t)out.tus.n;
       sp.ctu_intra_mask = 0;
       if (!pps.cu_qp_delta) { sp.qp_y_pred = sp.slice_qp; sp.cu_qp_delta_val = 0; }
       if (sh.sao_luma || sh.sao_chroma) {
@@ -1042,12 +1068,12 @@
       }
       if (sp.err) return sp.err;
       if (c.overrun()) return DEC_ERR_INVALID;
-      job.ctu[ctu].first = tu0;
-      job.ctu[ctu].count = ((uint32_t)out.tus.size() - tu0) | (sp.ctu_intra_mask << 24);
-      if (out.tus.size() - tu0 >= (1u << 24)) return DEC_ERR_INVALID;
+      job.ctu[ctu].first = out.tus.n != tu0 ? tu0 : tu0 - sub_tu0;
+      job.ctu[ctu].count = ((uint32_t)out.tus.n - tu0) | (sp.ctu_intra_mask << 24);
+      if (out.tus.n - tu0 >= (1u << 24)) return DEC_ERR_INVALID;
       if (wpp && cx == cx0 + 1) c.save_ctx(&job.wpp_saved[((size_t)cy * cols + g.tc) * CTX_COUNT]);
       if (((cut & 4) || scan) && wpp && free_slices && cx == cx1 - 1) c.save_ctx(&job.ds_saved[(size_t)cy * CTX_COUNT]);
-      if (wpp) job.row_progress[(size_t)cy * cols + g.tc].v.store(cx - cx0 + 1, std::memory_order_release);
+      if (wpp && !sequential) job.row_progress[(size_t)cy * cols + g.tc].v.store(cx - cx0 + 1, std::memory_order_release);
       const bool seg_last = free_slices ? (cut & 4) != 0 : cx == cx1 - 1 && (cols > 1 ? (cy == g.cy1 - 1 && job.seg_end_sub[(size_t)sub]) : job.seg_end_row[(size_t)cy] != 0);
       const int end = c.terminate();
       if (end != (seg_last ? 1 : 0)) {
@@ -1139,12 +1165,14 @@
       own->row_cols[(size_t)cy].store((uint8_t)own->cols, std::memory_order_release); own->row_done[(size_t)cy].store(1, std::memory_order_release);
     }
   };
+  const bool sequential = !(row_parallel && nsub > 1);
+  job.plain = plain_picture(job);
   auto one = [&](int r) {
     if (r >= nrecv) { skip_row(job.geom[(size_t)r].cy0); return; }
     if (band_nrows_ > 0 && (job.geom[(size_t)r].cy0 < band_row0_ || job.geom[(size_t)r].cy1 > band_row0_ + band_nrows_)) { job.subs[(size_t)r].rc = 0; return; }
     size_t start = job.sub_start[(size_t)r], end = (r + 1 < nrecv) ? job.sub_start[(size_t)r + 1] : len;
     if (scan_rows) { start = 0; end = len; }
-    int rc = end > start ? parse_substream(job, r, data + start, end - start, job.subs[(size_t)r]) : DEC_ERR_INVALID;
+    int rc = end > start ? parse_substream(job, r, data + start, end - start, job.subs[sequential ? 0 : (size_t)r], sequential) : DEC_ERR_INVALID;
     job.subs[(size_t)r].rc = rc;
     if (rc < 0 && job.pps.wpp) job.row_progress[(size_t)job.geom[(size_t)r].cy0 * cols + job.geom[(size_t)r].tc].v.store(1 << 30, std::memory_order_release);
     if (rc < 0) release_all();
@@ -1162,12 +1190,18 @@
   }
   size_t ntu = 0, nlev = 0;
   for (auto &r : job.subs) { if (r.rc < 0) return r.rc; ntu += r.tus.size(); nlev += r.levels.size(); }
+  if (job.plain) plain_pictures_.fetch_add(1, std::memory_order_relaxed);
   const bool bi = (job.sh.is_b || job.sh.weighted) && job.any_bi.load(std::memory_order_relaxed) != 0;
   const DecInputLayout lay = job.lay = DecInputLayout(pw_, ph_, ctbl_, ntu, nlev, job.b4x.size(), bi);
   if (!grow_job_input(job, lay.upload_bytes())) return DEC_ERR_GPU;
   if (bi) memcpy(job.h_in + lay.x_off, job.b4x.data(), lay.nb4x * sizeof(B4L1));
   DecTu *tus = (DecTu *)(job.h_in + lay.tu_off); uint32_t *lev = (uint32_t *)(job.h_in + lay.lev_off);
   size_t t = 0, l = 0;
+  if (sequential) {
+    const SubOut &so = job.subs[0];
+    if (ntu) memcpy(tus, so.tus.base, ntu * sizeof(DecTu));
+    if (nlev) memcpy(lev, so.levels.base, nlev * sizeof(uint32_t));
+  } else
   for (int r = 0; r < nsub; r++) {
     SubOut &so = job.subs[(size_t)r];
     const int cy0 = job.geom[(size_t)r].cy0, cy1 = job.geom[(size_t)r].cy1, cx0 = job.geom[(size_t)r].cx0, cx1 = job.geom[(size_t)r].cx1;
@@ -1177,8 +1211,8 @@
         if (ctbl_ == 6) for (int ry = 2 * cy; ry < 2 * cy + 2; ry++) for (int rx = 2 * cx0; rx < 2 * cx1; rx++) { TuRange &g = job.region[ry * 2 * wc + rx]; if (g.count) g.first += (uint32_t)t; }
       }
     }
-    for (DecTu td : so.tus) { td.offset += (uint32_t)l; tus[t++] = td; }
-    if (!so.levels.empty()) memcpy(lev + l, so.levels.data(), so.levels.size() * sizeof(uint32_t));
+    for (size_t k = 0; k < so.tus.n; k++) { DecTu td = so.tus.base[k]; td.offset += (uint32_t)l; tus[t++] = td; }
+    if (so.levels.n) memcpy(lev + l, so.levels.base, so.levels.n * sizeof(uint32_t));
     l += so.levels.size();
   }
   if (ctbl_ < 6) {
diff --git a/kvazzup_amd/csrc/decoder.h b/kvazzup_amd/csrc/decoder.h
--- a/kvazzup_amd/csrc/decoder.h
+++ b/kvazzup_amd/csrc/decoder.h
@@ -104,7 +104,26 @@
   void flush() {}
   int pending() const { return (int)(job_head_ - job_tail_) + (gpu_job_ ? 1 : 0) + (int)gpu_q_.size(); }
 
-  struct alignas(128) SubOut { std::vector<uint32_t> levels; std::vector<DecTu> tus; int rc = 0; };
+  template <class T> struct RawRun {
+    T *base = nullptr; size_t n = 0, cap = 0;
+    RawRun() {}
+    RawRun(RawRun &&o) noexcept : base(o.base), n(o.n), cap(o.cap) { o.base = nullptr; o.n = o.cap = 0; }
+    RawRun(const RawRun &) = delete; RawRun &operator=(const RawRun &) = delete;
+    ~RawRun() { free(base); }
+    void clear() { n = 0; }
+    size_t size() const { return n; }
+    __attribute__((noinline)) bool grow(size_t extra)
+    {
+      size_t want = cap ? cap * 2 : 64;
+      while (want < n + extra) want *= 2;
+      T *p = (T *)realloc((void *)base, want * sizeof(T));
+      if (!p) return false;
+      base = p; cap = want;
+      return true;
+    }
+    inline bool room(size_t extra) { return __builtin_expect(n + extra <= cap, 1) || grow(extra); }
+  };
+  struct alignas(128) SubOut { RawRun<uint32_t> levels; RawRun<DecTu> tus; int rc = 0; };
   struct alignas(64) Progress { std::atomic<int> v{0}; char pad[60]; };
   struct PicJob {
     std::vector<uint8_t> rbsp; size_t data_off = 0, data_len = 0;
@@ -141,6 +160,7 @@
     B4Rec *b4 = nullptr; TuRange *region = nullptr, *ctu = nullptr; uint8_t *ctu_tile = nullptr; SaoParams *sao = nullptr;
     std::vector<uint8_t> pred_mode, ct_depth, intra_mode;
     std::vector<SubOut> subs; std::vector<uint8_t> wpp_saved;
+    bool plain = false;
     std::unique_ptr<Progress[]> row_progress; int row_progress_n = 0;
     alignas(64) bool any_intra = false; bool any_inter = false;
     alignas(64) bool across_slices = true;
@@ -173,7 +193,11 @@
   int verify_hash(const PicJob &job, const std::vector<uint8_t> &want);
   bool check_hash_ = false; int hash_checked_ = 0, hash_mismatch_ = 0;
   int parse_job(PicJob &job, bool row_parallel);
-  int parse_substream(PicJob &job, int sub, const uint8_t *data, size_t len, SubOut &out);
+  int parse_substream(PicJob &job, int sub, const uint8_t *data, size_t len, SubOut &out, bool sequential);
+  template <bool PLAIN> int parse_substream_as(PicJob &job, int sub, const uint8_t *data, size_t len, SubOut &out, bool sequential);
+  bool plain_picture(const PicJob &job) const;
+  bool force_general_ = false;
+  std::atomic<uint32_t> plain_pictures_{0};
   int close_open_picture();
   int close_free_picture(PicJob &job);
   void take_back_job(PicJob &job); void file_damage(const PicJob &job); std::vector<uint8_t> layout_of(const PicJob &job) const; std::vector<uint8_t> damaged_layout_; uint32_t take_backs_ = 0;
diff --git a/kvazzup_amd/csrc/decoder.hip b/kvazzup_amd/csrc/decoder.hip
--- a/kvazzup_amd/csrc/decoder.hip
+++ b/kvazzup_amd/csrc/decoder.hip
@@ -63,6 +63,7 @@
 
 bool Decoder::start(std::string *error)
 {
+  { const char *e = getenv("KVAZZUP_AMD_PARSER_GENERAL"); force_general_ = e && atoi(e) != 0; }
   if (parse_only_) { frame_threads_ = 1; started_ = true; return true; }
   int ndev = 0;
   if (hipGetDeviceCount(&ndev) != hipSuccess || ndev <= device_) {
@@ -1433,6 +1434,7 @@
   if (w == "standin") { if (standin_slot_ < 0 || bytes > npx * 3 / 2) return false; return hipDeviceSynchronize() == hipSuccess && hipMemcpy(dst, dpb_[standin_slot_].plane[0], bytes, hipMemcpyDeviceToHost) == hipSuccess; }
   if (w == "standin_ms") { if (bytes != sizeof(float) || standin_ms_ < 0) return false; memcpy(dst, &standin_ms_, sizeof(float)); return true; }
   if (w == "take_backs") { if (bytes != sizeof(uint32_t)) return false; memcpy(dst, &take_backs_, sizeof(uint32_t)); return true; }
+  if (w == "plain_pictures") { if (bytes != sizeof(uint32_t)) return false; const uint32_t n = plain_pictures_.load(std::memory_order_relaxed); memcpy(dst, &n, sizeof(uint32_t)); return true; }
   if (w == "fill_mv") { if (fill_tab_.empty() || bytes > fill_tab_.size() * sizeof(int16_t)) return false; memcpy(dst, fill_tab_.data(), bytes); return true; }
   if (w == "partial_layout") {
     std::vector<uint8_t> lay = damaged_layout_;
```
